# SDFIdk/malstroem

Measured on AMD Instinct MI355X. Metric: Mcells/s fill->D8->accum->label on 16384^2 f32 DEM, higher is better.
Workload: dtype f32 fill / f64 no-flats+D8+accum / u8 flowdir / i32 labels; 1 GPU; 16384x16384 float32 DEM (spectral fBm beta=2 seed 42 (SURVEY 8d recipe)): fill+depths -> no-flats fill -> D8 -> accumulation -> CCL+label_stats -> watersheds+label_count -> pour points; parallelism=1 GPU, one device context, fill_rounds=8, noflat_rounds=84, fill_tiles=70225, fill_visits=44315, fill_cycles=0, noflat_visits=410496, noflat_cycles=410496, nlabels=4637017, fill_algorithm=1, fill_launches=8, noflat_algorithm=2, pour_algorithm=1

## Files before the change

### malstroem_amd/csrc/common.hpp

```cpp
#pragma once
#include <hip/hip_runtime.h>
#include <cstdint>
#include <cstdio>
#include <cstring>
#include <string>
#include <vector>

#include "../../include/malstroem_hip.h"

struct mhip_polygons;
struct mhip_flowpaths;

namespace mh {

void set_error(const char *fmt, ...);
const char *get_error();
const char *dev_env(const char *name);
hipError_t stream_sync(hipStream_t s);
int require_device();

#define MH_HIP(expr)                                                                             \
    do {                                                                                         \
        hipError_t _e = (expr);                                                                  \
        if (_e != hipSuccess) {                                                                  \
            mh::set_error("%s failed: %s (%s:%d)", #expr, hipGetErrorString(_e), __FILE__, __LINE__); \
            return MHIP_EHIP;                                                                    \
        }                                                                                        \
    } while (0)

#define MH_TRY(expr)                \
    do {                            \
        int _rc = (expr);           \
        if (_rc != MHIP_OK) return _rc; \
    } while (0)

#define MH_ARG(cond, msg)                   \
    do {                                    \
        if (!(cond)) {                      \
            mh::set_error("invalid argument: %s", msg); \
            return MHIP_EINVAL;             \
        }                                   \
    } while (0)

int pool_alloc(void **p, size_t bytes);
void pool_free(void *p, size_t bytes);

struct DevBuf {
    void *p = nullptr;
    size_t bytes = 0;
    DevBuf() = default;
    DevBuf(const DevBuf &) = delete;
    DevBuf &operator=(const DevBuf &) = delete;
    ~DevBuf() { release(); }
    int alloc(size_t n)
    {
        if (n == 0) n = 16;
        if (p && bytes >= n && bytes <= 2 * n + 4096) return MHIP_OK;
        release();
        MH_TRY(pool_alloc(&p, n));
        bytes = n;
        return MHIP_OK;
    }
    void release()
    {
        if (p) pool_free(p, bytes);
        p = nullptr;
        bytes = 0;
    }
    template <typename T> T *as() const { return reinterpret_cast<T *>(p); }
};

int upload(DevBuf &b, const void *host, size_t bytes, hipStream_t s);
int download(void *host, const DevBuf &b, size_t bytes, hipStream_t s);
int64_t build_rank_lut(const uint8_t *keep, int64_t nlab, std::vector<int32_t> &lut);
inline bool hyps_res_ok(double res) { return res > 0.0 && res <= 1.7976931348623157e308; }
int trace_on_device(const uint8_t *d_fd, const int32_t *d_lab, int64_t H, int64_t W, const int64_t *cells_rc, int64_t n, int use_bg,
                    int32_t bg, int32_t *out_label, int32_t *out_found, int64_t *out_len, const int64_t *offsets, int64_t *out_cells,
                    hipStream_t s);

__host__ __device__ inline int dir_dr(int k) { return (k == 0 || k == 1 || k == 7) ? -1 : (k >= 3 && k <= 5) ? 1 : 0; }
__host__ __device__ inline int dir_dc(int k) { return (k >= 1 && k <= 3) ? 1 : (k >= 5 && k <= 7) ? -1 : 0; }

__device__ __forceinline__ unsigned d8_code(double z, double u, double ur, double r, double dr, double d, double dl,
                                            double l, double ul)
{
    const double INV_SQRT2 = 0.7071067811865475;
    unsigned i = 8;
    double dzmax = 0.0, dz;
#define MH_D8_STEP(expr, k)          \
    dz = (expr);                     \
    i = dz > dzmax ? (k) : i;        \
    dzmax = fmax(dzmax, dz);
    MH_D8_STEP(__dsub_rn(z, u), 0u)
    MH_D8_STEP(__dmul_rn(__dsub_rn(z, ur), INV_SQRT2), 1u)
    MH_D8_STEP(__dsub_rn(z, r), 2u)
    MH_D8_STEP(__dmul_rn(__dsub_rn(z, dr), INV_SQRT2), 3u)
    MH_D8_STEP(__dsub_rn(z, d), 4u)
    MH_D8_STEP(__dmul_rn(__dsub_rn(z, dl), INV_SQRT2), 5u)
    MH_D8_STEP(__dsub_rn(z, l), 6u)
    MH_D8_STEP(__dmul_rn(__dsub_rn(z, ul), INV_SQRT2), 7u)
#undef MH_D8_STEP
    return i;
}

__device__ __forceinline__ unsigned edge_code(int64_t r, int64_t c, int64_t maxr, int64_t maxc)
{
    unsigned code = 8;
    if (r == 0) code = 0;
    if (r == maxr) code = 4;
    if (c == 0) code = 6;
    if (c == maxc) code = 2;
    if (r == 0 && c == 0) code = 7;
    if (r == 0 && c == maxc) code = 1;
    if (r == maxr && c == 0) code = 5;
    if (r == maxr && c == maxc) code = 3;
    return code;
}

__host__ __device__ inline uint32_t f32_key(float f)
{
    uint32_t u;
    memcpy(&u, &f, 4);
    return (u & 0x80000000u) ? ~u : (u | 0x80000000u);
}
__host__ __device__ inline float key_f32(uint32_t k)
{
    uint32_t u = (k & 0x80000000u) ? (k & 0x7fffffffu) : ~k;
    float f;
    memcpy(&f, &u, 4);
    return f;
}
__device__ __forceinline__ uint32_t dem_key(float v)
{
    if (v != v) return f32_key(__builtin_inff());
    return f32_key(v + 0.0f);
}
__host__ __device__ inline uint64_t f64_key(double f)
{
    uint64_t u;
    memcpy(&u, &f, 8);
    return (u & 0x8000000000000000ull) ? ~u : (u | 0x8000000000000000ull);
}
__host__ __device__ inline double key_f64(uint64_t k)
{
    uint64_t u = (k & 0x8000000000000000ull) ? (k & 0x7fffffffffffffffull) : ~k;
    double f;
    memcpy(&f, &u, 8);
    return f;
}

struct FillStats {
    int32_t rounds = 0;
    int64_t visits = 0;
    int64_t cycles = 0;
    int64_t tiles = 0;
    float hot_ms = 0;
    int32_t hot_launches = 0;
    int32_t algorithm = 0;
    uint32_t overflow = 0;
    bool have_minmax = false, dem_nan = false;
    float dem_min = 0.0f, dem_max = 0.0f;
    int32_t geo_reject = 0;
    int64_t geo_irregular = 0, geo_unreached = 0, geo_mismatch = 0;
};

struct FillRun {
    bool noflat = false;
    const float *dem = nullptr;
    void *out = nullptr;
    int64_t H = 0, W = 0;
    double sh = 0, dg = 0;
    const float *seed = nullptr;
    double seed_add = 0;
    int fixed_top = 0, fixed_bot = 0;
    int rounds_per_batch = 8;
    bool attach_only = false;
    struct Impl;
    Impl *impl;
    FillRun();
    ~FillRun();
    FillRun(const FillRun &) = delete;
    FillRun &operator=(const FillRun &) = delete;
    int begin(hipStream_t s, bool *active);
    int batch(hipStream_t s, bool *active);
    int activate_row(int side, hipStream_t s);
    int attach(hipStream_t s);
    int certify(hipStream_t s, bool *changed);
    int finish(hipStream_t s, FillStats *st);
};
void noflat_seed(FillRun &f, const float *d_filled, double sh, double dg, int64_t ncells_global);
struct PfRun;
struct FillHandover {
    PfRun *run = nullptr;
    const float *dem = nullptr;
    float *filled = nullptr, *depths = nullptr;
    int64_t H = 0, W = 0;
    const uint16_t *bslot = nullptr;
    const uint32_t *tabV = nullptr;
    int ntr = 0, ntc = 0;
    bool pending = false, queued = false, violated = false, repaired = false;
    bool suspect = false;
    unsigned long long *wet = nullptr;
    bool wet_ok = false;
    bool wet_pass = false;
    FillStats st_repair;
    FillHandover() = default;
    FillHandover(const FillHandover &) = delete;
    FillHandover &operator=(const FillHandover &) = delete;
    ~FillHandover();
    void release();
};
int fill_handover_complete(FillHandover *ho, hipStream_t s);
int fill_handover_repair(FillHandover *ho, hipStream_t s);
int fill_plain_dev(const float *d_dem, float *d_out, int64_t H, int64_t W, hipStream_t s, FillStats *st, float *d_depths = nullptr,
                   bool *depths_done = nullptr, FillHandover *ho = nullptr);
int fill_check_f32_dev(const float *d_dem, const float *d_filled, int64_t H, int64_t W, int fixed_top, int fixed_bot, hipStream_t s,
                       unsigned int *d_flag);
int fill_plain_pflood_dev(const float *d_dem, float *d_out, float *d_depths, int64_t H, int64_t W, hipStream_t s, FillStats *st, bool *violated = nullptr,
                          uint32_t *overflow = nullptr, FillHandover *ho = nullptr);
struct PfRun {
    const float *dem = nullptr;
    float *out = nullptr;
    int64_t H = 0, W = 0;
    int fixed_top = 0, fixed_bot = 0;
    uint32_t overflow = 0;
    struct Impl;
    Impl *impl;
    PfRun();
    ~PfRun();
    PfRun(const PfRun &) = delete;
    PfRun &operator=(const PfRun &) = delete;
    int begin(hipStream_t s);
    int halo_changed(int side, hipStream_t s);
    int batch(hipStream_t s);
    int finish(hipStream_t s, float *d_depths, FillStats *st, bool *violated = nullptr, FillHandover *ho = nullptr);
    int finish_late(hipStream_t s, float *d_depths, bool *violated);
    int proof_flag(hipStream_t s, unsigned int *h_flag);
    int solve(hipStream_t s);
    int pack(hipStream_t s, int row0, int nrows);
    int publish_edges(hipStream_t s);
};
struct StageHook {
    enum Point { FIRST_VISIT = 0, TAIL_ROUNDS = 1, FINISH = 3 };
    void (*fn)(void *, hipStream_t) = nullptr;
    void *arg = nullptr;
    bool fired = false;
    int at = TAIL_ROUNDS;
    void fire(hipStream_t s)
    {
        if (fn && !fired) {
            fired = true;
            fn(arg, s);
        }
    }
    void fire_at(int point, hipStream_t s)
    {
        if (point == at) fire(s);
    }
};

struct GeoRun {
    const float *dem = nullptr, *filled = nullptr;
    double *out = nullptr;
    uint32_t *dist = nullptr;
    int64_t H = 0, W = 0;
    double sh = 0, dg = 0;
    int fixed_top = 0, fixed_bot = 0;
    bool allow_partial = false;
    double seed_add = 0;
    bool partial = false;
    StageHook *tail_hook = nullptr;
    uint8_t *d8_out = nullptr;
    unsigned int *d8_nodir = nullptr;
    bool d8_done = false;
    bool defer_out = false;
    bool out_deferred = false;
    FillHandover *handover = nullptr;
    bool wet_used = false;
    struct Impl;
    Impl *impl;
    GeoRun();
    ~GeoRun();
    GeoRun(const GeoRun &) = delete;
    GeoRun &operator=(const GeoRun &) = delete;
    int begin(hipStream_t s, bool *applicable, bool *active);
    int batch(hipStream_t s, bool *active);
    int halo_changed(int side, hipStream_t s);
    int end(hipStream_t s, bool *ok, FillStats *st);
    int launch_rounds(hipStream_t s, int nb);
};
struct D8Sink {
    uint8_t *flowdir = nullptr;
    unsigned int *nodir = nullptr;
    bool done = false;
    uint32_t *dist = nullptr;
    bool defer = false, deferred = false;
};
int noflat_assemble_dev(const float *d_filled, const uint32_t *d_dist, double *d_out, int64_t n, double seed_add, hipStream_t s);
int fill_noflat_geodesic_dev(const float *d_dem, const float *d_filled, double *d_out, int64_t H, int64_t W, double sh, double dg, double seed_add,
                             hipStream_t s, FillStats *st, bool *partial, StageHook *tail_hook = nullptr, D8Sink *d8 = nullptr, FillHandover *ho = nullptr);
int noflat_verify_dev(const float *d_dem, const double *d_out, int64_t H, int64_t W, double sh, double dg, hipStream_t s, bool *ok, int fixed_top = 0,
                      int fixed_bot = 0);
int fill_noflat_dev(const float *d_dem, double *d_out, int64_t H, int64_t W, double sh, double dg, hipStream_t s,
                    FillStats *st = nullptr, const float *d_filled = nullptr, StageHook *tail_hook = nullptr, D8Sink *d8 = nullptr,
                    FillHandover *ho = nullptr);
int short_diag_dev(const float *d_dem, int64_t n, double *sh, double *dg, hipStream_t s);
int depths_dev(const float *d_filled, const float *d_dem, float *d_out, int64_t n, hipStream_t s);
int d8_dev(const double *d_z, uint8_t *d_out, int64_t H, int64_t W, int edges_outward, hipStream_t s, int64_t row_off = 0,
           int64_t Hg = 0, unsigned int *d_interior_nodir = nullptr);
void short_diag_from_minmax(float mn, float mx, bool has_nan, double *sh, double *dg);
int minmax_dev(const float *d_x, int64_t n, float *mn, float *mx, int *has_nan, hipStream_t s);
int row_update_dev(void *d_dst, const void *d_src, int64_t nbytes, int *changed, hipStream_t s);
int copy_bandwidth_dev(size_t bytes, int reps, double *gbs, hipStream_t s);
int read_bandwidth_dev(size_t bytes, int reps, double *gbs, hipStream_t s);
int row_update_async(void *d_dst, const void *d_src, int64_t nbytes, int *d_changed, hipStream_t s);
int trace_downstream_dev(const uint8_t *d_fd, const int32_t *d_lab, int64_t H, int64_t W, const int64_t *d_cells, int64_t n, int use_bg,
// ... 278 lines not shown
```

### malstroem_amd/csrc/ctx.hip

```cpp
#include <mutex>
#include <new>
#include <string>
#include <vector>

#include "ctx.hpp"

namespace mh {

static void drop_hyps(mhip_ctx *c)
{
    c->hyps_total = -1;
    c->have[MHIP_R_FINALDEPTHS] = false;
    c->wetat_events = -1;
    c->wetat_out.release();
}

static void drop_flow_distance(mhip_ctx *c)
{
    std::lock_guard<std::mutex> lk(c->fdist_mu);
    c->fdist_unresolved = -1;
    c->fdist_out.release();
    c->fdist_rec.release();
}

// ... 300 lines not shown
int mhip_ctx_upload_dem(mhip_ctx *c, const float *dem) { return mhip_ctx_upload(c, MHIP_R_DEM, dem); }

int mhip_ctx_upload_rows(mhip_ctx *c, int which, int64_t row0, int64_t nrows, const void *host)
{
    MH_ARG(c && host && which >= 0 && which < MHIP_R_COUNT_ && row0 >= 0 && nrows >= 1 && row0 + nrows <= c->H_owned,
           "ctx_upload_rows(ctx, which, row0, nrows, host)");
    MH_HIP(hipSetDevice(c->device));
    MH_TRY(ctx_raster(c, which));
    MH_TRY(ctx_settle(c, which, true));
    ctx_wrote(c, which, true);
    c->have[which] = false;
    MH_TRY(ctx_copy_rows(c, c->r[which].p, raster_elem(which), row0, nrows, const_cast<void *>(host), hipMemcpyHostToDevice));
    if (row0 + nrows == c->H_owned) {
        c->have[which] = true;
        if (which == MHIP_R_LABELS) c->labels_filtered = true;
    }
    return MHIP_OK;
}

int mhip_ctx_download_rows(mhip_ctx *c, int which, int64_t row0, int64_t nrows, void *host)
{
    MH_ARG(c && host && which >= 0 && which < MHIP_R_COUNT_ && row0 >= 0 && nrows >= 1 && row0 + nrows <= c->H_owned,
           "ctx_download_rows(ctx, which, row0, nrows, host)");
    MH_ARG(c->have[which], "raster has not been computed or uploaded");
    MH_TRY(ctx_settle(c, which, false));
    return ctx_copy_rows(c, c->r[which].p, raster_elem(which), row0, nrows, host, hipMemcpyDeviceToHost);
}

int mhip_ctx_download(mhip_ctx *c, int which, void *host)
{
    MH_ARG(c && host && which >= 0 && which < MHIP_R_COUNT_, "ctx_download(ctx, which, host)");
    return mhip_ctx_download_rows(c, which, 0, c->H_owned, host);
}

int mhip_ctx_trace_downstream(mhip_ctx *c, const int64_t *cells_rc, int64_t n, int use_background, int32_t background, int32_t *out_label,
                              int32_t *out_found, int64_t *out_len, const int64_t *offsets, int64_t *out_cells)
{
    MH_ARG(c && n >= 0 && (n == 0 || cells_rc), "ctx_trace_downstream(ctx, cells, n, ...)");
    MH_ARG(c->have[MHIP_R_FLOWDIR] && c->have[MHIP_R_LABELS], "ctx_trace_downstream needs flow directions and labels");
    MH_ARG(!c->ht && !c->hb, "stream tracing runs on an undivided raster");
    if (n == 0) return MHIP_OK;
    MH_HIP(hipSetDevice(c->device));
    return trace_on_device(c->r[MHIP_R_FLOWDIR].as<uint8_t>(), c->r[MHIP_R_LABELS].as<int32_t>(), c->H, c->W, cells_rc, n, use_background,
                           background, out_label, out_found, out_len, offsets, out_cells, c->stream);
}

int mhip_ctx_sync(mhip_ctx *c)
{
    MH_ARG(c, "ctx");
    MH_HIP(stream_sync(c->stream));
    return MHIP_OK;
}

int mhip_ctx_stage_ms(mhip_ctx *c, int stage, float *ms)
{
    MH_ARG(c && ms, "ctx_stage_ms(ctx, stage, ms)");
    const int k = timer_slot(stage);
    MH_ARG(k >= 0 && c->timers[k].valid, "stage has not been run");
    MH_HIP(hipEventSynchronize(c->timers[k].b));
    MH_HIP(hipEventElapsedTime(ms, c->timers[k].a, c->timers[k].b));
    return MHIP_OK;
}

int mhip_ctx_kernel_ms(mhip_ctx *c, const char *kernel, float *ms_total, int32_t *launches)
{
    MH_ARG(c && kernel && ms_total && launches, "ctx_kernel_ms(ctx, kernel, ms, launches)");
    const std::string k(kernel);
    if (k == "d8") {
        *launches = 1;
        return mhip_ctx_stage_ms(c, MHIP_STAGE_FLOWDIR, ms_total);
    }
    if (k == "d8_steady") {
        MH_ARG(c->have[MHIP_R_NOFLAT] && !c->ht && !c->hb, "d8_steady needs the no-flats surface on an undivided context");
        MH_HIP(hipSetDevice(c->device));
        double *g = nullptr;
        MH_TRY(ctx_noflat(c, &g));
        MH_TRY(ctx_raster(c, MHIP_R_FLOWDIR));
        MH_TRY(c->nodir_cnt.alloc(4));
        constexpr int REPS = 16;
        StageTimer *t;
        MH_TRY(ctx_timer(c, D8_STEADY_SLOT, &t));
        hipStream_t s = c->stream;
        ctx_wrote(c, MHIP_R_FLOWDIR);
        MH_HIP(hipMemsetAsync(c->nodir_cnt.p, 0, 4, s));
        for (int i = 0; i < REPS + 2; ++i) {
            if (i == 2) MH_HIP(hipEventRecord(t->a, s));
            MH_TRY(d8_dev(g, c->r[MHIP_R_FLOWDIR].as<uint8_t>(), c->H, c->W, 1, s, 0, c->H_global, c->nodir_cnt.as<unsigned int>()));
        }
        MH_HIP(hipEventRecord(t->b, s));
        MH_HIP(hipEventSynchronize(t->b));
        MH_HIP(hipEventElapsedTime(ms_total, t->a, t->b));
        c->have[MHIP_R_FLOWDIR] = true;
        c->nodir_valid = true;
        c->flowdir_own = true;
        *launches = REPS;
        return MHIP_OK;
    }
    if (k == "hyps_table" || k == "final_depths") {
        *launches = 1;
        return mhip_ctx_stage_ms(c, k == "hyps_table" ? HYPS_KERNEL_SLOT : FINAL_KERNEL_SLOT, ms_total);
    }
    if (k == "wet_at") {
        *launches = 1;
        return mhip_ctx_stage_ms(c, WETAT_KERNEL_SLOT, ms_total);
    }
    if (k == "fill_round") {
        *launches = c->fill_rounds;
        return mhip_ctx_stage_ms(c, MHIP_STAGE_FILL, ms_total);
    }
    if (k == "noflat_round") {
        *launches = c->noflat_rounds;
        return mhip_ctx_stage_ms(c, MHIP_STAGE_NOFLAT, ms_total);
    }
    set_error("unknown kernel family '%s'", kernel);
    return MHIP_EINVAL;
}

int mhip_ctx_get_i64(mhip_ctx *c, const char *key, int64_t *value)
{
    MH_ARG(c && key && value, "ctx_get_i64(ctx, key, value)");
    const std::string k(key);
    if (k == "nlabels_raw") *value = c->nlabels_raw;
    else if (k == "nlabels") {
        if (c->nlabels < 0 && c->have[MHIP_R_LABELS]) {
            MH_HIP(hipSetDevice(c->device));
            MH_TRY(ctx_label_max(c, c->stream));
        }
        *value = c->nlabels;
    }
    else if (k == "fill_rounds") *value = c->fill_rounds;
    else if (k == "noflat_rounds") *value = c->noflat_rounds;
    else if (k == "fill_visits") *value = c->fill_st.visits;
    else if (k == "fill_cycles") *value = c->fill_st.cycles;
    else if (k == "fill_tiles") *value = c->fill_st.tiles;
    else if (k == "fill_algorithm") *value = c->fill_st.algorithm;
    else if (k == "fill_handover") *value = c->fill_handover;
    else if (k == "wetbits_used") *value = (c->wet_pass_used ? 1 : 0) | (c->wet_label_used ? 2 : 0);
    else if (k == "fill_handover_rechecks") *value = c->fill_handover_rechecks;
    else if (k == "fill_overflow") *value = c->fill_st.overflow;
    else if (k == "fill_launches") *value = c->fill_st.rounds;
    else if (k == "fill_hot_launches") *value = c->fill_st.hot_launches;
    else if (k == "noflat_hot_launches") *value = c->noflat_st.hot_launches;
    else if (k == "accum_algorithm") *value = c->accum_algorithm;
    else if (k == "flowdir_computed") *value = (c->have[MHIP_R_FLOWDIR] && c->flowdir_own) ? 1 : 0;
    else if (k == "pour_algorithm") *value = c->pour_algorithm;
    else if (k == "noflat_algorithm") *value = c->noflat_st.algorithm;
    else if (k == "noflat_pending") *value = c->noflat_pending ? 1 : 0;
    else if (k == "noflat_visits") *value = c->noflat_st.visits;
    else if (k == "noflat_reject") *value = c->noflat_st.geo_reject;
    else if (k == "noflat_reject_irregular") *value = c->noflat_st.geo_irregular;
    else if (k == "noflat_reject_unreached") *value = c->noflat_st.geo_unreached;
    else if (k == "noflat_reject_mismatch") *value = c->noflat_st.geo_mismatch;
    else if (k == "noflat_cycles") *value = c->noflat_st.cycles;
    else if (k == "hyps_bins") *value = c->hyps_total;
    else if (k == "hyps_lds_spills") *value = c->hyps_spills;
    else if (k == "wet_at_events") *value = c->wetat_events;
    else if (k == "flow_distance_unresolved") *value = c->fdist_unresolved;
    else if (k == "hand_undrained") *value = c->hand_undrained;
    else if (k == "reach_catchments") *value = c->rcatch_nreach;
    else if (k == "inundation") *value = c->inund_held;
    else if (k == "zones") *value = c->nzone;
    else if (k == "H") *value = c->H;
    else if (k == "W") *value = c->W;
    else {
        set_error("unknown key '%s'", key);
        return MHIP_EINVAL;
    }
    return MHIP_OK;
}

int mhip_ctx_get_f64(mhip_ctx *c, const char *key, double *value)
{
    MH_ARG(c && key && value, "ctx_get_f64(ctx, key, value)");
    const std::string k(key);
    if (k == "short") *value = c->sh;
    else if (k == "diag") *value = c->dg;
    else if (k == "fill_hot_ms") *value = c->fill_st.hot_ms;
    else if (k == "noflat_hot_ms") *value = c->noflat_st.hot_ms;
    else {
        set_error("unknown key '%s'", key);
        return MHIP_EINVAL;
    }
    return MHIP_OK;
}

int mhip_ctx_raw_stats(mhip_ctx *c, mhip_stat_record *records)
{
    MH_ARG(c && records && c->raw_stats.p && c->nlabels_raw >= 0, "ctx_raw_stats needs a LABEL run");
    return ctx_fetch(c, c->raw_stats, sizeof(mhip_stat_record) * (size_t)(c->nlabels_raw + 1), records);
}

int mhip_ctx_apply_keep(mhip_ctx *c, const uint8_t *keep)
{
    MH_ARG(c, "ctx");
    MH_HIP(hipSetDevice(c->device));
    return ctx_apply_keep_on(c, keep, c->stream);
}

int mhip_ctx_stats(mhip_ctx *c, mhip_stat_record *records)
{
    MH_ARG(c && records && c->stats_valid && c->labels_filtered, "ctx_stats needs LABEL + apply_keep (or mhip_ctx_hyps) on the resident depths and labels");
    return ctx_fetch(c, c->stats, sizeof(mhip_stat_record) * (size_t)(c->nlabels + 1), records);
}

int mhip_ctx_watershed_counts(mhip_ctx *c, int64_t *counts)
{
    MH_ARG(c && counts && c->ws_counts_valid, "ctx_watershed_counts needs a WATERSHED run on the resident labels");
    return ctx_fetch(c, c->ws_counts, 8 * (size_t)(c->nlabels + 1), counts);
}

int mhip_ctx_pourpoints(mhip_ctx *c, mhip_index_record *records)
{
    MH_ARG(c && records && c->pour_valid, "ctx_pourpoints needs a POURPOINTS run on the resident labels and accumulated flow");
    return ctx_fetch(c, c->pour, sizeof(mhip_index_record) * (size_t)(c->nlabels + 1), records);
}

int mhip_ctx_hyps(mhip_ctx *c, double res, int64_t *total)
{
    MH_ARG(c && total && hyps_res_ok(res), "ctx_hyps(ctx, 0 < res < inf, total)");
    MH_ARG(!(c->nranks > 1 || c->ht || c->hb), "hypsometry on a row band is not built (the tables of the bands add up: a later step); use an undivided context");
    MH_ARG(c->have[MHIP_R_DEPTHS] && c->have[MHIP_R_LABELS] && !c->ccl_pending, "ctx_hyps needs the DEPTHS and LABELS rasters");
    MH_ARG(c->labels_filtered, "ctx_hyps needs mhip_ctx_apply_keep after the LABEL run");
    MH_HIP(hipSetDevice(c->device));
    hipStream_t s = c->stream;
    const int64_t n = c->H * c->W;
    c->hyps_total = -1;
    if (!c->stats_valid) {
        MH_TRY(ctx_label_max(c, s));
        MH_TRY(c->stats.alloc(sizeof(mhip_stat_record) * (size_t)(c->nlabels + 1)));
        MH_TRY(label_stats_dev(c->r[MHIP_R_DEPTHS].as<float>(), c->r[MHIP_R_LABELS].as<int32_t>(), n, c->nlabels, c->stats.as<mhip_stat_record>(), s,
                               c->W, c->labels_components));
        c->stats_valid = true;
    }
    const int64_t nlab = c->nlabels;
    MH_TRY(c->hyps_off.alloc(8 * (size_t)(nlab + 2)));
    StageTimer *k;
    MH_TRY(ctx_timer(c, HYPS_KERNEL_SLOT, &k));
    MH_TRY(stage_begin(c, MHIP_STAGE_HYPS, s));
    int64_t tot = 0;
    MH_TRY(hyps_layout_dev(c->stats.as<double>() + 1, 4, nlab, res, c->hyps_off.as<int64_t>(), &tot, s));
    MH_TRY(c->hyps_cnt.alloc(4 * (size_t)tot));
    MH_TRY(c->hyps_sum.alloc(8 * (size_t)tot));
    MH_TRY(hyps_table_dev(c->r[MHIP_R_DEPTHS].as<float>(), c->r[MHIP_R_LABELS].as<int32_t>(), n, c->W, nlab, res, c->hyps_off.as<int64_t>(), tot,
                          c->hyps_cnt.as<uint32_t>(), c->hyps_sum.as<double>(), &c->hyps_spills, s, k->a, k->b));
    MH_TRY(stage_end(c, MHIP_STAGE_HYPS, s));
    k->valid = true;
    c->hyps_total = tot;
    *total = tot;
    return MHIP_OK;
}

int mhip_ctx_hyps_fetch(mhip_ctx *c, int64_t *offsets, int64_t *counts, double *sums)
{
    MH_ARG(c && offsets && counts && sums, "ctx_hyps_fetch(ctx, offsets, counts, sums)");
    MH_ARG(c->hyps_total >= 0, "ctx_hyps_fetch needs mhip_ctx_hyps on the resident depths and labels");
    MH_HIP(hipSetDevice(c->device));
    hipStream_t s = c->stream;
    const size_t tot = (size_t)c->hyps_total;
    std::vector<uint32_t> c32(tot + 1);
    MH_HIP(hipMemcpyAsync(offsets, c->hyps_off.p, 8 * (size_t)(c->nlabels + 2), hipMemcpyDeviceToHost, s));
    if (tot) {
        MH_HIP(hipMemcpyAsync(c32.data(), c->hyps_cnt.p, 4 * tot, hipMemcpyDeviceToHost, s));
        MH_HIP(hipMemcpyAsync(sums, c->hyps_sum.p, 8 * tot, hipMemcpyDeviceToHost, s));
    }
    MH_HIP(stream_sync(s));
    for (size_t k = 0; k < tot; ++k) counts[k] = (int64_t)c32[k];
    return MHIP_OK;
}

int mhip_ctx_final_depths(mhip_ctx *c, const double *q, mhip_final_record *records)
{
    MH_ARG(c && q && records, "ctx_final_depths(ctx, q, records)");
    MH_ARG(c->hyps_total >= 0 && c->stats_valid, "ctx_final_depths needs mhip_ctx_hyps on the resident depths and labels");
    MH_HIP(hipSetDevice(c->device));
    hipStream_t s = c->stream;
    const int64_t nlab = c->nlabels, n = c->H * c->W;
    DevBuf d_q;
    MH_TRY(upload(d_q, q, 8 * (size_t)(nlab + 1), s));
    MH_TRY(c->hyps_rec.alloc(sizeof(mhip_final_record) * (size_t)(nlab + 1)));
    MH_TRY(ctx_raster(c, MHIP_R_FINALDEPTHS));
    c->have[MHIP_R_FINALDEPTHS] = false;
    StageTimer *k;
    MH_TRY(ctx_timer(c, FINAL_KERNEL_SLOT, &k));
    MH_TRY(stage_begin(c, MHIP_STAGE_FINALDEPTHS, s));
    MH_TRY(hyps_levels_dev(nlab, c->hyps_off.as<int64_t>(), c->hyps_cnt.as<uint32_t>(), c->hyps_sum.as<double>(), c->stats.as<double>() + 1, 4,
                           d_q.as<double>(), c->hyps_rec.as<mhip_final_record>(), s));
    MH_TRY(final_depths_dev(c->r[MHIP_R_DEPTHS].as<float>(), c->r[MHIP_R_LABELS].as<int32_t>(), n, c->W, nlab, c->hyps_rec.as<mhip_final_record>(),
                            c->r[MHIP_R_FINALDEPTHS].as<float>(), s, k->a, k->b));
    MH_TRY(stage_end(c, MHIP_STAGE_FINALDEPTHS, s));
    k->valid = true;
    c->have[MHIP_R_FINALDEPTHS] = true;
    return ctx_fetch(c, c->hyps_rec, sizeof(mhip_final_record) * (size_t)(nlab + 1), records);
}

int mhip_ctx_wet_at(mhip_ctx *c, int32_t K, const double *q, const float *values, mhip_final_record *records)
{
    MH_ARG(c && q && values && records, "ctx_wet_at(ctx, K, q, values, records)");
    MH_ARG(wet_at_events_ok(K, values), "ctx_wet_at: 1 to 16 events whose values are finite, > 0 and strictly increasing");
    MH_ARG(!(c->nranks > 1 || c->ht || c->hb), "wet_at on a row band is not built (it needs the bands' hypsometry tables: a later step); use an undivided context");
    MH_ARG(c->hyps_total >= 0 && c->stats_valid, "ctx_wet_at needs mhip_ctx_hyps on the resident depths and labels");
    MH_HIP(hipSetDevice(c->device));
    hipStream_t s = c->stream;
    const int64_t nlab = c->nlabels, n = c->H * c->W;
    const size_t nt = (size_t)K * (size_t)(nlab + 1);
    DevBuf d_q, d_rec;
    MH_TRY(upload(d_q, q, 8 * nt, s));
// ... 277 lines not shown
```

### malstroem_amd/csrc/noflat_geo.hip

```cpp
#include <algorithm>
#include <cmath>
#include <cstdlib>
#include <mutex>
#include <string>
#include <type_traits>
#include <vector>

#include "common.hpp"
#include "handover_addr.hpp"

namespace mh {

namespace {

constexpr int WN = 64;
constexpr int TI = 62;
constexpr uint32_t DINF = 0xE0000000u;
constexpr uint32_t WMAX = 1u << 28;
constexpr uint32_t D_IRR = 0xFFFFFFFFu;
constexpr uint32_t M_NOFLAT = 0xFF00u;
constexpr uint32_t M_IRR = 0xFD00u;
constexpr uint32_t M_WALL = 0xFE00u;
constexpr int DPP_WF_SL1 = 0x130;
constexpr int DPP_WF_SR1 = 0x138;
#ifndef NG_MAXCYC
#define NG_MAXCYC 1
#endif
enum { C_IRREGULAR = 0, C_UNREACHED = 1, C_MISMATCH = 2, C_FATAL = 3, C_PROOF = 4, C_STATS = 8 };
static_assert(WN == ho::WN && TI == ho::TI, "handover_addr.hpp cuts the raster like this file");

__device__ __forceinline__ uint32_t from_left(uint32_t v) { return (uint32_t)__builtin_amdgcn_update_dpp(0, (int)v, DPP_WF_SR1, 0xf, 0xf, true); }
__device__ __forceinline__ uint32_t from_right(uint32_t v) { return (uint32_t)__builtin_amdgcn_update_dpp(0, (int)v, DPP_WF_SL1, 0xf, 0xf, true); }

__device__ __forceinline__ float fleft(float v)
{
    return __int_as_float(__builtin_amdgcn_update_dpp(0x7f800000, __float_as_int(v), DPP_WF_SR1, 0xf, 0xf, false));
}
__device__ __forceinline__ float fright(float v)
{
    return __int_as_float(__builtin_amdgcn_update_dpp(0x7f800000, __float_as_int(v), DPP_WF_SL1, 0xf, 0xf, false));
}

__device__ __forceinline__ uint32_t class_above(float V)
{
    const uint32_t b = __float_as_uint(V), ex = (b >> 23) & 0xffu;
    const uint32_t e = ((b >> 31) && (b & 0x7fffffu) == 0u) ? ex - 1u : ex;
    return (ex == 0u || ex == 255u) ? 255u : e;
}
__device__ __forceinline__ double class_ulp(uint32_t e) { return __longlong_as_double((long long)(e + 1023u - 127u - 52u) << 52); }

struct GeoArgs {
    int64_t H, W;
    int ntr, ntc, nt;
    const float *F;
    uint32_t *d;
    uint32_t *blk;
    uint32_t *hdr;
    uint8_t *mark;
    const int *list;
    const uint32_t *count;
    const uint32_t *tab;
    unsigned long long *counters;
    int maxcyc;
    int append, round_next;
    int *amark;
    int *list_next;
    uint32_t *count_next;
    int fixed_top, fixed_bot;
    const float *ho_dem;
    const uint16_t *ho_bslot;
    const uint32_t *ho_tabV;
    float *ho_F, *ho_depths;
    unsigned long long *ho_wet;
};

template <int R> __device__ __forceinline__ void lds_put(uint32_t addr, uint32_t v) { asm volatile("ds_write_b32 %0, %1 offset:%2" : : "v"(addr), "v"(v), "n"(R) : "memory"); }
template <int R> __device__ __forceinline__ uint32_t lds_get(uint32_t addr)
{
    uint32_t v;
    asm volatile("ds_read_b32 %0, %1 offset:%2" : "=v"(v) : "v"(addr), "n"(R) : "memory");
    return v;
}
__device__ __forceinline__ void lds_wait() { asm volatile("s_waitcnt lgkmcnt(0)" : : : "memory"); }
template <int R0, int N> __device__ __forceinline__ void lds_put_rows(uint32_t addr, const uint32_t (&x)[WN])
{
    if constexpr (N > 0) {
        lds_put<R0 * (WN + 1) * 4>(addr, x[R0]);
        lds_put_rows<R0 + 1, N - 1>(addr, x);
    }
}
template <int R0, int N> __device__ __forceinline__ void lds_get_rows(uint32_t addr, uint32_t (&x)[WN])
{
    if constexpr (N > 0) {
        x[R0] = lds_get<R0 * (WN + 1) * 4>(addr);
        lds_get_rows<R0 + 1, N - 1>(addr, x);
    }
}
template <int C0, int N> __device__ __forceinline__ void lds_get_cols(uint32_t addr, uint32_t (&x)[WN])
{
    if constexpr (N > 0) {
        x[C0] = lds_get<C0 * 4>(addr);
        lds_get_cols<C0 + 1, N - 1>(addr, x);
    }
}
__device__ __forceinline__ void transpose32(uint32_t (&x)[WN], uint32_t scr_b, int lane)
{
    lds_put_rows<0, WN>(scr_b + 4u * lane, x);
    lds_wait();
    lds_get_cols<0, WN>(scr_b + 4u * (WN + 1) * lane, x);
    lds_wait();
#pragma unroll
    for (int c = 0; c < WN; ++c) asm volatile("" : "+v"(x[c]));
}

struct LaneW {
    __device__ __forceinline__ void get(uint32_t mword, const uint32_t *tab_l, uint32_t &s, uint32_t &g) const
    {
        const uint32_t e = (mword >> 8) & 0xffu;
        s = tab_l[e];
        g = tab_l[256 + e];
    }
};

template <bool DOWN, typename WT>
__device__ __forceinline__ void pass(uint32_t (&d)[WN], uint32_t (&ni)[WN], const WT wt, const uint32_t *tab_l, uint32_t &acc_all,
                                     uint32_t &acc_first, uint32_t &acc_last)
{
    constexpr int first = DOWN ? 1 : TI, dir = DOWN ? 1 : -1;
    constexpr int bC = DOWN ? 0 : 4, bL = DOWN ? 7 : 5, bR = DOWN ? 1 : 3;
#pragma unroll
    for (int r = 0; r < WN; ++r) asm volatile("" : "+v"(d[r]), "+v"(ni[r]));
#pragma unroll
    for (int i = 0; i < TI; ++i) {
        const int r = first + dir * i;
        const uint32_t behind = d[r - dir];
        const uint32_t bl = from_left(behind), br = from_right(behind);
        const uint32_t w = ni[r];
        uint32_t S, G;
        wt.get(w, tab_l, S, G);
        const uint32_t c0 = (behind + S) | (uint32_t)__builtin_amdgcn_sbfe((int)w, bC, 1);
        const uint32_t c1 = (bl + G) | (uint32_t)__builtin_amdgcn_sbfe((int)w, bL, 1);
        const uint32_t c2 = (br + G) | (uint32_t)__builtin_amdgcn_sbfe((int)w, bR, 1);
        const uint32_t cu = d[r];
        const uint32_t nv = min(min(c0, c1), min(c2, cu));
        const uint32_t x = nv ^ cu;
        acc_all |= x;
        asm volatile("" : "+v"(acc_all));
        if (r == 1) acc_first |= (w & 0x83u) != 0x83u ? x : 0u;
        if (r == TI) acc_last |= (w & 0x38u) != 0x38u ? x : 0u;
        d[r] = nv;
        __builtin_amdgcn_sched_barrier(0);
    }
}

template <typename WT>
__device__ __forceinline__ void relax(uint32_t (&d)[WN], uint32_t (&ni)[WN], const WT wt, const uint32_t *tab_l, uint32_t scr_b, int lane, int maxcyc,
                                      unsigned &wake, bool &changed, bool &capped, unsigned &cycles)
{
    const uint64_t INNER = ((1ull << TI) - 1) << 1, B1 = 2ull, B62 = 1ull << TI;
    capped = true;
#pragma nounroll
    for (int cyc = 0; cyc < maxcyc; ++cyc) {
        uint64_t chg = 0;
        ++cycles;
#pragma nounroll
        for (int half = 0; half < 2; ++half) {
            uint32_t acc_all = 0, acc_first = 0, acc_last = 0;
            pass<true>(d, ni, wt, tab_l, acc_all, acc_first, acc_last);
            pass<false>(d, ni, wt, tab_l, acc_all, acc_first, acc_last);
            const uint64_t all = __ballot(acc_all != 0), fst = __ballot(acc_first != 0), lst = __ballot(acc_last != 0);
            chg |= all;
            const unsigned e_first = (fst & INNER) ? 1u : 0u, e_last = (lst & INNER) ? 1u : 0u;
            const unsigned l1 = (all & B1) ? 1u : 0u, l62 = (all & B62) ? 1u : 0u;
            const unsigned f1 = (fst & B1) ? 1u : 0u, f62 = (fst & B62) ? 1u : 0u, g1 = (lst & B1) ? 1u : 0u, g62 = (lst & B62) ? 1u : 0u;
            if (half == 0)
                wake |= (e_first << 1) | (e_last << 7) | (l1 << 3) | (l62 << 5) | (f1 << 0) | (f62 << 2) | (g1 << 6) | (g62 << 8);
            else
                wake |= (e_first << 3) | (e_last << 5) | (l1 << 1) | (l62 << 7) | (f1 << 0) | (f62 << 6) | (g1 << 2) | (g62 << 8);
            transpose32(d, scr_b, lane);
#pragma unroll
            for (int r = 0; r < WN; ++r) ni[r] = __builtin_amdgcn_alignbit(ni[r], ni[r], 16);
        }
        changed |= chg != 0;
        if (!chg) {
            capped = false;
            break;
        }
    }
}

constexpr int NMK = 9;
#define NG_DPP " row_mask:0xf bank_mask:0xf bound_ctrl:1\n\t"
#define NG_ROW(O, I, B, BIT)                                                                                                                 \
    "v_add_u32 %[u], %[" B "], %[S]\n\t"                                                                                                    \
    "v_add_u32_dpp %[t], %[" B "], %[G] wave_shr:1" NG_DPP                                                                                   \
    "v_add_u32_dpp %[k], %[" B "], %[G] wave_shl:1" NG_DPP                                                                                   \
    "v_min3_u32 %[t], %[u], %[t], %[k]\n\t"                                                                                                 \
    "v_bfe_i32 %[k], %[m], " BIT ", 1\n\t"                                                                                                  \
    "v_min_u32 %[" O "], %[t], %[" I "]\n\t"                                                                                                \
    "v_bfi_b32 %[" O "], %[k], %[" I "], %[" O "]\n\t"                                                                                      \
    "v_bitop3_b32 %[acc], %[" O "], %[acc], %[" I "] bitop3:0xde\n\t"
template <int R, int DIR>
__device__ __forceinline__ void rows6_wl(uint32_t (&d)[WN], const uint32_t m, const uint32_t S, const uint32_t G, uint32_t &acc)
{
    static_assert((R >> 5) == ((R + 5 * DIR) >> 5), "one mask word a block");
    uint32_t o0, o1, o2, o3, o4, o5, u, t, k;
    if constexpr (DIR > 0)
        asm volatile(NG_ROW("o0", "i0", "b", "%[bit]") NG_ROW("o1", "i1", "o0", "%[bit]+1") NG_ROW("o2", "i2", "o1", "%[bit]+2")
                     NG_ROW("o3", "i3", "o2", "%[bit]+3") NG_ROW("o4", "i4", "o3", "%[bit]+4") NG_ROW("o5", "i5", "o4", "%[bit]+5")
                     : [o0] "=&v"(o0), [o1] "=&v"(o1), [o2] "=&v"(o2), [o3] "=&v"(o3), [o4] "=&v"(o4), [o5] "=&v"(o5), [u] "=&v"(u), [t] "=&v"(t),
                       [k] "=&v"(k), [acc] "+v"(acc)
                     : [b] "v"(d[R - DIR]), [i0] "v"(d[R]), [i1] "v"(d[R + DIR]), [i2] "v"(d[R + 2 * DIR]), [i3] "v"(d[R + 3 * DIR]),
                       [i4] "v"(d[R + 4 * DIR]), [i5] "v"(d[R + 5 * DIR]), [S] "v"(S), [G] "v"(G), [m] "v"(m), [bit] "n"(R & 31));
    else
        asm volatile(NG_ROW("o0", "i0", "b", "%[bit]") NG_ROW("o1", "i1", "o0", "%[bit]-1") NG_ROW("o2", "i2", "o1", "%[bit]-2")
                     NG_ROW("o3", "i3", "o2", "%[bit]-3") NG_ROW("o4", "i4", "o3", "%[bit]-4") NG_ROW("o5", "i5", "o4", "%[bit]-5")
                     : [o0] "=&v"(o0), [o1] "=&v"(o1), [o2] "=&v"(o2), [o3] "=&v"(o3), [o4] "=&v"(o4), [o5] "=&v"(o5), [u] "=&v"(u), [t] "=&v"(t),
                       [k] "=&v"(k), [acc] "+v"(acc)
                     : [b] "v"(d[R - DIR]), [i0] "v"(d[R]), [i1] "v"(d[R + DIR]), [i2] "v"(d[R + 2 * DIR]), [i3] "v"(d[R + 3 * DIR]),
                       [i4] "v"(d[R + 4 * DIR]), [i5] "v"(d[R + 5 * DIR]), [S] "v"(S), [G] "v"(G), [m] "v"(m), [bit] "n"(R & 31));
    d[R] = o0; d[R + DIR] = o1; d[R + 2 * DIR] = o2; d[R + 3 * DIR] = o3; d[R + 4 * DIR] = o4; d[R + 5 * DIR] = o5;
}
template <int R, int DIR>
__device__ __forceinline__ uint32_t row1_wl(uint32_t (&d)[WN], const uint32_t m, const uint32_t S, const uint32_t G, uint32_t &acc)
{
    uint32_t o0, u, t, k;
    const uint32_t cu = d[R];
    asm volatile("s_nop 1\n\t" NG_ROW("o0", "i0", "b", "%[bit]") "s_nop 1"
                 : [o0] "=&v"(o0), [u] "=&v"(u), [t] "=&v"(t), [k] "=&v"(k), [acc] "+v"(acc)
                 : [b] "v"(d[R - DIR]), [i0] "v"(cu), [S] "v"(S), [G] "v"(G), [m] "v"(m), [bit] "n"(R & 31));
    d[R] = o0;
    return o0 ^ cu;
}
template <int R, int DIR, int N>
__device__ __forceinline__ void blocks_wl(uint32_t (&d)[WN], const uint32_t lo, const uint32_t hi, const uint32_t S, const uint32_t G, uint32_t &acc)
{
    if constexpr (N > 0) {
        rows6_wl<R, DIR>(d, R < 32 ? lo : hi, S, G, acc);
        __builtin_amdgcn_sched_barrier(0);
        blocks_wl<R + 6 * DIR, DIR, N - 1>(d, lo, hi, S, G, acc);
    }
}
template <bool DOWN>
__device__ __forceinline__ void pass_wl(uint32_t (&d)[WN], const uint32_t imm_lo, const uint32_t imm_hi, const uint32_t S, const uint32_t G,
                                        const bool edge_first, const bool edge_last, uint32_t &acc_all, uint32_t &acc_first, uint32_t &acc_last)
{
#pragma unroll
    for (int r = 0; r < WN; ++r) asm volatile("" : "+v"(d[r]));
    uint32_t lo = imm_lo, hi = imm_hi;
    asm volatile("" : "+v"(lo), "+v"(hi));
    if constexpr (DOWN) {
        const uint32_t x1 = row1_wl<1, 1>(d, lo, S, G, acc_all);
        acc_first |= edge_first ? x1 : 0u;
        __builtin_amdgcn_sched_barrier(0);
        blocks_wl<2, 1, 10>(d, lo, hi, S, G, acc_all);
        const uint32_t x2 = row1_wl<TI, 1>(d, hi, S, G, acc_all);
        acc_last |= edge_last ? x2 : 0u;
    } else {
        const uint32_t x2 = row1_wl<TI, -1>(d, hi, S, G, acc_all);
        acc_last |= edge_last ? x2 : 0u;
        __builtin_amdgcn_sched_barrier(0);
        blocks_wl<TI - 1, -1, 10>(d, lo, hi, S, G, acc_all);
        const uint32_t x1 = row1_wl<1, -1>(d, lo, S, G, acc_all);
        acc_first |= edge_first ? x1 : 0u;
    }
    __builtin_amdgcn_sched_barrier(0);
}

__device__ __forceinline__ void relax_wl(uint32_t (&d)[WN], const uint32_t (&mk)[13], const uint32_t S, const uint32_t G, uint32_t scr_b, int lane, int maxcyc,
                                         unsigned &wake, bool &changed, bool &capped, unsigned &cycles)
{
    const uint64_t INNER = ((1ull << TI) - 1) << 1, B1 = 2ull, B62 = 1ull << TI;
    capped = true;
#pragma nounroll
    for (int cyc = 0; cyc < maxcyc; ++cyc) {
        uint64_t chg = 0;
        ++cycles;
        {
            uint32_t acc_all = 0, acc_first = 0, acc_last = 0;
            pass_wl<true>(d, mk[0], mk[1], S, G, (mk[8] & 1u) != 0u, (mk[8] & 2u) != 0u, acc_all, acc_first, acc_last);
            pass_wl<false>(d, mk[0], mk[1], S, G, (mk[8] & 1u) != 0u, (mk[8] & 2u) != 0u, acc_all, acc_first, acc_last);
            const uint64_t all = __ballot(acc_all != 0), fst = __ballot(acc_first != 0), lst = __ballot(acc_last != 0);
            chg |= all;
            const unsigned e_first = (fst & INNER) ? 1u : 0u, e_last = (lst & INNER) ? 1u : 0u;
            const unsigned l1 = (all & B1) ? 1u : 0u, l62 = (all & B62) ? 1u : 0u;
            const unsigned f1 = (fst & B1) ? 1u : 0u, f62 = (fst & B62) ? 1u : 0u, g1 = (lst & B1) ? 1u : 0u, g62 = (lst & B62) ? 1u : 0u;
            wake |= (e_first << 1) | (e_last << 7) | (l1 << 3) | (l62 << 5) | (f1 << 0) | (f62 << 2) | (g1 << 6) | (g62 << 8);
            transpose32(d, scr_b, lane);
        }
        {
            uint32_t acc_all = 0, acc_first = 0, acc_last = 0;
            pass_wl<true>(d, mk[4], mk[5], S, G, (mk[8] & 4u) != 0u, (mk[8] & 8u) != 0u, acc_all, acc_first, acc_last);
            pass_wl<false>(d, mk[4], mk[5], S, G, (mk[8] & 4u) != 0u, (mk[8] & 8u) != 0u, acc_all, acc_first, acc_last);
            const uint64_t all = __ballot(acc_all != 0), fst = __ballot(acc_first != 0), lst = __ballot(acc_last != 0);
            chg |= all;
            const unsigned e_first = (fst & INNER) ? 1u : 0u, e_last = (lst & INNER) ? 1u : 0u;
            const unsigned l1 = (all & B1) ? 1u : 0u, l62 = (all & B62) ? 1u : 0u;
            const unsigned f1 = (fst & B1) ? 1u : 0u, f62 = (fst & B62) ? 1u : 0u, g1 = (lst & B1) ? 1u : 0u, g62 = (lst & B62) ? 1u : 0u;
            wake |= (e_first << 3) | (e_last << 5) | (l1 << 1) | (l62 << 7) | (f1 << 0) | (f62 << 6) | (g1 << 2) | (g62 << 8);
            transpose32(d, scr_b, lane);
        }
        changed |= chg != 0;
        if (!chg) {
            capped = false;
            break;
        }
    }
}

constexpr int NMK2 = 13;
#define NG_ROW2(O, I, B, BIT)                                                                                                                \
    "v_bfe_i32 %[k], %[c], " BIT ", 1\n\t"                                                                                                  \
    "v_bfi_b32 %[g], %[k], %[G2], %[G1]\n\t"                                                                                                \
    "v_bfi_b32 %[s], %[k], %[S2], %[S1]\n\t"                                                                                                \
    "v_add_u32 %[u], %[" B "], %[s]\n\t"                                                                                                    \
    "v_add_u32_dpp %[t], %[" B "], %[g] wave_shr:1" NG_DPP                                                                                   \
    "v_add_u32_dpp %[k], %[" B "], %[g] wave_shl:1" NG_DPP                                                                                   \
    "v_min3_u32 %[t], %[u], %[t], %[k]\n\t"                                                                                                 \
    "v_bfe_i32 %[k], %[m], " BIT ", 1\n\t"                                                                                                  \
    "v_min_u32 %[" O "], %[t], %[" I "]\n\t"                                                                                                \
    "v_bfi_b32 %[" O "], %[k], %[" I "], %[" O "]\n\t"                                                                                      \
    "v_bitop3_b32 %[acc], %[" O "], %[acc], %[" I "] bitop3:0xde\n\t"
struct TwoWeights {
    uint32_t S1, G1, S2, G2;
};
template <int R, int DIR>
__device__ __forceinline__ void rows6_wl2(uint32_t (&d)[WN], const uint32_t m, const uint32_t c, const TwoWeights w, uint32_t &acc)
{
    static_assert((R >> 5) == ((R + 5 * DIR) >> 5), "one mask word a block");
    uint32_t o0, o1, o2, o3, o4, o5, u, t, k, sw, gw;
    if constexpr (DIR > 0)
        asm volatile(NG_ROW2("o0", "i0", "b", "%[bit]") NG_ROW2("o1", "i1", "o0", "%[bit]+1") NG_ROW2("o2", "i2", "o1", "%[bit]+2")
                     NG_ROW2("o3", "i3", "o2", "%[bit]+3") NG_ROW2("o4", "i4", "o3", "%[bit]+4") NG_ROW2("o5", "i5", "o4", "%[bit]+5")
                     : [o0] "=&v"(o0), [o1] "=&v"(o1), [o2] "=&v"(o2), [o3] "=&v"(o3), [o4] "=&v"(o4), [o5] "=&v"(o5), [u] "=&v"(u), [t] "=&v"(t),
                       [k] "=&v"(k), [s] "=&v"(sw), [g] "=&v"(gw), [acc] "+v"(acc)
                     : [b] "v"(d[R - DIR]), [i0] "v"(d[R]), [i1] "v"(d[R + DIR]), [i2] "v"(d[R + 2 * DIR]), [i3] "v"(d[R + 3 * DIR]),
                       [i4] "v"(d[R + 4 * DIR]), [i5] "v"(d[R + 5 * DIR]), [S1] "v"(w.S1), [G1] "v"(w.G1), [S2] "v"(w.S2), [G2] "v"(w.G2), [m] "v"(m),
                       [c] "v"(c), [bit] "n"(R & 31));
    else
        asm volatile(NG_ROW2("o0", "i0", "b", "%[bit]") NG_ROW2("o1", "i1", "o0", "%[bit]-1") NG_ROW2("o2", "i2", "o1", "%[bit]-2")
                     NG_ROW2("o3", "i3", "o2", "%[bit]-3") NG_ROW2("o4", "i4", "o3", "%[bit]-4") NG_ROW2("o5", "i5", "o4", "%[bit]-5")
                     : [o0] "=&v"(o0), [o1] "=&v"(o1), [o2] "=&v"(o2), [o3] "=&v"(o3), [o4] "=&v"(o4), [o5] "=&v"(o5), [u] "=&v"(u), [t] "=&v"(t),
                       [k] "=&v"(k), [s] "=&v"(sw), [g] "=&v"(gw), [acc] "+v"(acc)
                     : [b] "v"(d[R - DIR]), [i0] "v"(d[R]), [i1] "v"(d[R + DIR]), [i2] "v"(d[R + 2 * DIR]), [i3] "v"(d[R + 3 * DIR]),
                       [i4] "v"(d[R + 4 * DIR]), [i5] "v"(d[R + 5 * DIR]), [S1] "v"(w.S1), [G1] "v"(w.G1), [S2] "v"(w.S2), [G2] "v"(w.G2), [m] "v"(m),
                       [c] "v"(c), [bit] "n"(R & 31));
    d[R] = o0; d[R + DIR] = o1; d[R + 2 * DIR] = o2; d[R + 3 * DIR] = o3; d[R + 4 * DIR] = o4; d[R + 5 * DIR] = o5;
}
template <int R, int DIR>
__device__ __forceinline__ uint32_t row1_wl2(uint32_t (&d)[WN], const uint32_t m, const uint32_t c, const TwoWeights w, uint32_t &acc)
{
    uint32_t o0, u, t, k, sw, gw;
    const uint32_t cu = d[R];
    asm volatile("s_nop 1\n\t" NG_ROW2("o0", "i0", "b", "%[bit]") "s_nop 1"
                 : [o0] "=&v"(o0), [u] "=&v"(u), [t] "=&v"(t), [k] "=&v"(k), [s] "=&v"(sw), [g] "=&v"(gw), [acc] "+v"(acc)
                 : [b] "v"(d[R - DIR]), [i0] "v"(cu), [S1] "v"(w.S1), [G1] "v"(w.G1), [S2] "v"(w.S2), [G2] "v"(w.G2), [m] "v"(m), [c] "v"(c),
                   [bit] "n"(R & 31));
    d[R] = o0;
    return o0 ^ cu;
}
template <int R, int DIR, int N>
__device__ __forceinline__ void blocks_wl2(uint32_t (&d)[WN], const uint32_t lo, const uint32_t hi, const uint32_t clo, const uint32_t chi, const TwoWeights w,
                                           uint32_t &acc)
{
    if constexpr (N > 0) {
        rows6_wl2<R, DIR>(d, R < 32 ? lo : hi, R < 32 ? clo : chi, w, acc);
        __builtin_amdgcn_sched_barrier(0);
        blocks_wl2<R + 6 * DIR, DIR, N - 1>(d, lo, hi, clo, chi, w, acc);
    }
}
template <bool DOWN>
__device__ __forceinline__ void pass_wl2(uint32_t (&d)[WN], const uint32_t imm_lo, const uint32_t imm_hi, const uint32_t cls_lo, const uint32_t cls_hi,
                                         const TwoWeights w, const bool edge_first, const bool edge_last, uint32_t &acc_all, uint32_t &acc_first,
                                         uint32_t &acc_last)
{
#pragma unroll
    for (int r = 0; r < WN; ++r) asm volatile("" : "+v"(d[r]));
    uint32_t lo = imm_lo, hi = imm_hi, clo = cls_lo, chi = cls_hi;
    asm volatile("" : "+v"(lo), "+v"(hi), "+v"(clo), "+v"(chi));
    if constexpr (DOWN) {
        const uint32_t x1 = row1_wl2<1, 1>(d, lo, clo, w, acc_all);
        acc_first |= edge_first ? x1 : 0u;
        __builtin_amdgcn_sched_barrier(0);
        blocks_wl2<2, 1, 10>(d, lo, hi, clo, chi, w, acc_all);
        const uint32_t x2 = row1_wl2<TI, 1>(d, hi, chi, w, acc_all);
        acc_last |= edge_last ? x2 : 0u;
    } else {
        const uint32_t x2 = row1_wl2<TI, -1>(d, hi, chi, w, acc_all);
        acc_last |= edge_last ? x2 : 0u;
        __builtin_amdgcn_sched_barrier(0);
        blocks_wl2<TI - 1, -1, 10>(d, lo, hi, clo, chi, w, acc_all);
        const uint32_t x1 = row1_wl2<1, -1>(d, lo, clo, w, acc_all);
        acc_first |= edge_first ? x1 : 0u;
    }
    __builtin_amdgcn_sched_barrier(0);
}
__device__ __forceinline__ void relax_wl2(uint32_t (&d)[WN], const uint32_t (&mk)[NMK2], const TwoWeights w, uint32_t scr_b, int lane, int maxcyc, unsigned &wake,
                                          bool &changed, bool &capped, unsigned &cycles)
{
    const uint64_t INNER = ((1ull << TI) - 1) << 1, B1 = 2ull, B62 = 1ull << TI;
    capped = true;
#pragma nounroll
    for (int cyc = 0; cyc < maxcyc; ++cyc) {
        uint64_t chg = 0;
        ++cycles;
        {
            uint32_t acc_all = 0, acc_first = 0, acc_last = 0;
            pass_wl2<true>(d, mk[0], mk[1], mk[9], mk[10], w, (mk[8] & 1u) != 0u, (mk[8] & 2u) != 0u, acc_all, acc_first, acc_last);
            pass_wl2<false>(d, mk[0], mk[1], mk[9], mk[10], w, (mk[8] & 1u) != 0u, (mk[8] & 2u) != 0u, acc_all, acc_first, acc_last);
            const uint64_t all = __ballot(acc_all != 0), fst = __ballot(acc_first != 0), lst = __ballot(acc_last != 0);
            chg |= all;
            const unsigned e_first = (fst & INNER) ? 1u : 0u, e_last = (lst & INNER) ? 1u : 0u;
            const unsigned l1 = (all & B1) ? 1u : 0u, l62 = (all & B62) ? 1u : 0u;
            const unsigned f1 = (fst & B1) ? 1u : 0u, f62 = (fst & B62) ? 1u : 0u, g1 = (lst & B1) ? 1u : 0u, g62 = (lst & B62) ? 1u : 0u;
            wake |= (e_first << 1) | (e_last << 7) | (l1 << 3) | (l62 << 5) | (f1 << 0) | (f62 << 2) | (g1 << 6) | (g62 << 8);
            transpose32(d, scr_b, lane);
        }
        {
            uint32_t acc_all = 0, acc_first = 0, acc_last = 0;
            pass_wl2<true>(d, mk[4], mk[5], mk[11], mk[12], w, (mk[8] & 4u) != 0u, (mk[8] & 8u) != 0u, acc_all, acc_first, acc_last);
            pass_wl2<false>(d, mk[4], mk[5], mk[11], mk[12], w, (mk[8] & 4u) != 0u, (mk[8] & 8u) != 0u, acc_all, acc_first, acc_last);
            const uint64_t all = __ballot(acc_all != 0), fst = __ballot(acc_first != 0), lst = __ballot(acc_last != 0);
            chg |= all;
            const unsigned e_first = (fst & INNER) ? 1u : 0u, e_last = (lst & INNER) ? 1u : 0u;
            const unsigned l1 = (all & B1) ? 1u : 0u, l62 = (all & B62) ? 1u : 0u;
            const unsigned f1 = (fst & B1) ? 1u : 0u, f62 = (fst & B62) ? 1u : 0u, g1 = (lst & B1) ? 1u : 0u, g62 = (lst & B62) ? 1u : 0u;
            wake |= (e_first << 3) | (e_last << 5) | (l1 << 1) | (l62 << 7) | (f1 << 0) | (f62 << 6) | (g1 << 2) | (g62 << 8);
            transpose32(d, scr_b, lane);
        }
        changed |= chg != 0;
        if (!chg) {
            capped = false;
            break;
        }
    }
}

#define NG_ROW_OPEN(O, I, B)                                                                                                                 \
    "v_add_u32 %[u], %[" B "], %[S]\n\t"                                                                                                    \
    "v_add_u32_dpp %[t], %[" B "], %[G] wave_shr:1" NG_DPP                                                                                   \
    "v_add_u32_dpp %[k], %[" B "], %[G] wave_shl:1" NG_DPP                                                                                   \
    "v_min3_u32 %[t], %[u], %[t], %[k]\n\t"                                                                                                 \
    "v_min_u32 %[" O "], %[t], %[" I "]\n\t"                                                                                                \
    "v_cndmask_b32_e64 %[" O "], %[" O "], %[" I "], %[ring]\n\t"                                                                            \
    "v_bitop3_b32 %[acc], %[" O "], %[acc], %[" I "] bitop3:0xde\n\t"
template <int R, int DIR>
__device__ __forceinline__ void rows6_open(uint32_t (&d)[WN], const uint64_t ring, const uint32_t S, const uint32_t G, uint32_t &acc)
{
    uint32_t o0, o1, o2, o3, o4, o5, u, t, k;
    asm volatile(NG_ROW_OPEN("o0", "i0", "b") NG_ROW_OPEN("o1", "i1", "o0") NG_ROW_OPEN("o2", "i2", "o1") NG_ROW_OPEN("o3", "i3", "o2")
                 NG_ROW_OPEN("o4", "i4", "o3") NG_ROW_OPEN("o5", "i5", "o4")
                 : [o0] "=&v"(o0), [o1] "=&v"(o1), [o2] "=&v"(o2), [o3] "=&v"(o3), [o4] "=&v"(o4), [o5] "=&v"(o5), [u] "=&v"(u), [t] "=&v"(t), [k] "=&v"(k),
                   [acc] "+v"(acc)
                 : [b] "v"(d[R - DIR]), [i0] "v"(d[R]), [i1] "v"(d[R + DIR]), [i2] "v"(d[R + 2 * DIR]), [i3] "v"(d[R + 3 * DIR]), [i4] "v"(d[R + 4 * DIR]),
                   [i5] "v"(d[R + 5 * DIR]), [S] "v"(S), [G] "v"(G), [ring] "s"(ring));
    d[R] = o0; d[R + DIR] = o1; d[R + 2 * DIR] = o2; d[R + 3 * DIR] = o3; d[R + 4 * DIR] = o4; d[R + 5 * DIR] = o5;
}
template <int R, int DIR>
__device__ __forceinline__ uint32_t row1_open(uint32_t (&d)[WN], const uint64_t ring, const uint32_t S, const uint32_t G, uint32_t &acc)
{
    uint32_t o0, u, t, k;
    const uint32_t cu = d[R];
    asm volatile("s_nop 1\n\t" NG_ROW_OPEN("o0", "i0", "b") "s_nop 1"
                 : [o0] "=&v"(o0), [u] "=&v"(u), [t] "=&v"(t), [k] "=&v"(k), [acc] "+v"(acc)
                 : [b] "v"(d[R - DIR]), [i0] "v"(cu), [S] "v"(S), [G] "v"(G), [ring] "s"(ring));
    d[R] = o0;
    return o0 ^ cu;
}
template <int R, int DIR, int N>
__device__ __forceinline__ void blocks_open(uint32_t (&d)[WN], const uint64_t ring, const uint32_t S, const uint32_t G, uint32_t &acc)
{
    if constexpr (N > 0) {
        rows6_open<R, DIR>(d, ring, S, G, acc);
        __builtin_amdgcn_sched_barrier(0);
        blocks_open<R + 6 * DIR, DIR, N - 1>(d, ring, S, G, acc);
    }
}
template <bool DOWN>
__device__ __forceinline__ void pass_open(uint32_t (&d)[WN], const uint32_t S, const uint32_t G, const bool ring_lane, uint32_t &acc_all, uint32_t &acc_first,
                                          uint32_t &acc_last)
{
#pragma unroll
    for (int r = 0; r < WN; ++r) asm volatile("" : "+v"(d[r]));
    const uint64_t ring = __ballot(ring_lane);
    if constexpr (DOWN) {
        acc_first |= row1_open<1, 1>(d, ring, S, G, acc_all);
        __builtin_amdgcn_sched_barrier(0);
        blocks_open<2, 1, 10>(d, ring, S, G, acc_all);
        acc_last |= row1_open<TI, 1>(d, ring, S, G, acc_all);
    } else {
        acc_last |= row1_open<TI, -1>(d, ring, S, G, acc_all);
        __builtin_amdgcn_sched_barrier(0);
        blocks_open<TI - 1, -1, 10>(d, ring, S, G, acc_all);
        acc_first |= row1_open<1, -1>(d, ring, S, G, acc_all);
    }
    __builtin_amdgcn_sched_barrier(0);
}

__device__ __forceinline__ void relax_open(uint32_t (&d)[WN], const uint32_t S, const uint32_t G, uint32_t scr_b, int lane, int maxcyc, unsigned &wake,
                                           bool &changed, bool &capped, unsigned &cycles)
{
    const uint64_t INNER = ((1ull << TI) - 1) << 1, B1 = 2ull, B62 = 1ull << TI;
    const bool ring_lane = (lane == 0) | (lane == WN - 1);
    capped = true;
#pragma nounroll
    for (int cyc = 0; cyc < maxcyc; ++cyc) {
        uint64_t chg = 0;
        ++cycles;
#pragma nounroll
        for (int half = 0; half < 2; ++half) {
            uint32_t acc_all = 0, acc_first = 0, acc_last = 0;
            pass_open<true>(d, S, G, ring_lane, acc_all, acc_first, acc_last);
            pass_open<false>(d, S, G, ring_lane, acc_all, acc_first, acc_last);
            const uint64_t all = __ballot(acc_all != 0), fst = __ballot(acc_first != 0), lst = __ballot(acc_last != 0);
            chg |= all;
            const unsigned e_first = (fst & INNER) ? 1u : 0u, e_last = (lst & INNER) ? 1u : 0u;
            const unsigned l1 = (all & B1) ? 1u : 0u, l62 = (all & B62) ? 1u : 0u;
            const unsigned f1 = (fst & B1) ? 1u : 0u, f62 = (fst & B62) ? 1u : 0u, g1 = (lst & B1) ? 1u : 0u, g62 = (lst & B62) ? 1u : 0u;
            if (half == 0) wake |= (e_first << 1) | (e_last << 7) | (l1 << 3) | (l62 << 5) | (f1 << 0) | (f62 << 2) | (g1 << 6) | (g62 << 8);
            else wake |= (e_first << 3) | (e_last << 5) | (l1 << 1) | (l62 << 7) | (f1 << 0) | (f62 << 6) | (g1 << 2) | (g62 << 8);
            transpose32(d, scr_b, lane);
        }
        changed |= chg != 0;
        if (!chg) {
            capped = false;
            break;
        }
    }
}

constexpr uint32_t HDR_ACTIVE = 1u << 31, HDR_UNIFORM = 1u << 9, HDR_OPEN = 1u << 10, HDR_TWO = 1u << 11;
template <bool FIRST, bool HANDOVER = false>
__device__ __forceinline__ void visit(const GeoArgs &a, int t, const uint32_t *tab_l, uint32_t scr_b, int lane, unsigned &visits, unsigned &cycles)
{
#ifdef NG_PROFILE
    const long long tp0 = __builtin_amdgcn_s_memtime();
#endif
    const int64_t H = a.H, W = a.W;
    const int ti = t / a.ntc, tj = t - ti * a.ntc;
    const int64_t r0 = (int64_t)ti * TI, c0 = (int64_t)tj * TI;
    const int64_t cc = c0 + lane;
    const bool col_in = cc < W;
    const uint32_t lane_c = (uint32_t)(col_in ? lane : W - 1 - c0);

    const int64_t org = r0 * W + c0;
    const __amdgpu_buffer_rsrc_t rd = __builtin_amdgcn_make_buffer_rsrc((void *)(a.d + org), 0, 0x7fffffff, 0x00020000);
    const __amdgpu_buffer_rsrc_t rb = __builtin_amdgcn_make_buffer_rsrc((void *)(a.blk + (int64_t)t * (WN * WN)), 0, WN * WN * 4, 0x00020000);
    int Wi = (int)W;
    asm volatile("" : "+s"(Wi));
    const int last_row = (int)(H - 1 - r0 < WN - 1 ? H - 1 - r0 : WN - 1);
    uint32_t ni[WN], d[WN], mk[NMK2];
    uint32_t hdr;
    if constexpr (FIRST) {
        const __amdgpu_buffer_rsrc_t rf = __builtin_amdgcn_make_buffer_rsrc((void *)(a.F + org), 0, 0x7fffffff, 0x00020000);
        const bool ring_lane = (lane == 0) | (lane == WN - 1);
        const bool lane_in = (lane >= 1) & (lane <= TI) & (cc < W - 1);
        const bool lane_border = (tj == 0 && lane == 0) | (cc >= W - 1);
        const float PINF = __builtin_inff();
        const int border_row = (int)(H - 1 - r0 < 2 * WN ? H - 1 - r0 : 2 * WN);
        uint32_t lake_any = 0, nirr = 0, nfatal = 0;
        uint32_t proof_bad = 0;
        auto classify = [&](auto inner_tag) {
            constexpr bool INNER = decltype(inner_tag)::value;
            const bool lane_in_c = INNER ? ((lane >= 1) & (lane <= TI)) : lane_in;
            float f[WN];
            uint32_t raised[2] = {0u, 0u};
            if constexpr (!HANDOVER) {
                int so = 0;
#pragma unroll
                for (int r = 0; r < WN; ++r) {
                    f[r] = __uint_as_float(__builtin_amdgcn_raw_buffer_load_b32(rf, (int)((INNER ? (uint32_t)lane : lane_c) * 4u), INNER ? r * Wi * 4 : so * 4, 0));
                    so = r < last_row ? so + Wi : so;
                }
            } else {
                const ho::Win w = ho::window(H, W, a.ntr, a.ntc, ti, tj);
                const int64_t tab0 = ho::tab_origin(w), tab_left = ho::tab_words_behind_origin(w) * 4;
                const __amdgpu_buffer_rsrc_t re = __builtin_amdgcn_make_buffer_rsrc((void *)(a.ho_dem + org), 0, 0x7fffffff, 0x00020000);
                const __amdgpu_buffer_rsrc_t rs = __builtin_amdgcn_make_buffer_rsrc((void *)(a.ho_bslot + org), 0, 0x7fffffff, 0x00020000);
                const __amdgpu_buffer_rsrc_t rt =
                    __builtin_amdgcn_make_buffer_rsrc((void *)(a.ho_tabV + tab0), 0, (int)(tab_left < 0x7fffffff ? tab_left : 0x7fffffff), 0x00020000);
                const __amdgpu_buffer_rsrc_t rF = __builtin_amdgcn_make_buffer_rsrc((void *)(a.ho_F + org), 0, 0x7fffffff, 0x00020000);
                const __amdgpu_buffer_rsrc_t rD =
                    __builtin_amdgcn_make_buffer_rsrc((void *)(a.ho_depths ? a.ho_depths + org : a.ho_F), 0, a.ho_depths ? 0x7fffffff : 0, 0x00020000);
                const uint32_t col_read = INNER ? (uint32_t)lane : (uint32_t)ho::col_of(w, lane);
                const bool bcol = INNER ? false : ho::border_col(w, lane);
                const uint32_t lane_bytes = ho::tab_lane_words(w, lane) * 4u;
                const int row_bytes_top = (int)(ho::tab_row_words(w, 0) * 4u), row_bytes_mid = (int)(ho::tab_row_words(w, 1) * 4u),
                          row_bytes_bot = (int)(ho::tab_row_words(w, WN - 1) * 4u);
                const bool ocol = INNER ? lane_in_c : ho::own_col(w, lane);
                volatile __attribute__((address_space(3))) uint32_t *const scr_p = (volatile __attribute__((address_space(3))) uint32_t *)(uintptr_t)scr_b + lane;
                uint32_t below = 0u;
                constexpr int QR = 16;
                uint32_t sl[WN];
                auto load_q = [&](int q) {
#pragma unroll
                    for (int r = q * QR; r < (q + 1) * QR; ++r) {
                        const int so = INNER ? r * Wi : (r < last_row ? r : last_row) * Wi;
                        f[r] = __uint_as_float(__builtin_amdgcn_raw_buffer_load_b32(re, (int)(col_read * 4u), so * 4, 0));
                        sl[r] = (uint32_t)(uint16_t)__builtin_amdgcn_raw_buffer_load_b16(rs, (int)(col_read * 2u), so * 2, 0);
                    }
                    __builtin_amdgcn_sched_barrier(0);
                };
                auto gather_q = [&](int q) {
#pragma unroll
                    for (int r = q * QR; r < (q + 1) * QR; ++r) {
                        const bool border = INNER ? false : (bcol | ho::border_row(w, r));
                        sl[r] = __builtin_amdgcn_raw_buffer_load_b32(rt, (int)(lane_bytes + ho::tab_slot(sl[r], border) * 4u),
                                                                     r == 0 ? row_bytes_top : (r == WN - 1 ? row_bytes_bot : row_bytes_mid), 0);
                    }
                    __builtin_amdgcn_sched_barrier(0);
                };
                auto finish_q = [&](int q) {
#pragma unroll
                    for (int r = q * QR; r < (q + 1) * QR; ++r) {
                        const bool border = INNER ? false : (bcol | ho::border_row(w, r));
                        const float e = f[r];
                        const float lev = key_f32(max(dem_key(e), sl[r]));
                        const float v = border ? e : lev;
                        raised[r >> 5] |= v > e ? 1u << (r & 31) : 0u;
                        below |= v < e ? 1u : 0u;
                        asm volatile("" : "+v"(below), "+v"(raised[r >> 5]));
                        if ((INNER ? (r >= 1 && r <= TI) : ho::own_row(w, r)) && ocol) {
                            __builtin_amdgcn_raw_buffer_store_b32(__float_as_uint(v), rF, lane * 4, r * Wi * 4, 0);
                            __builtin_amdgcn_raw_buffer_store_b32(__float_as_uint(v - e), rD, lane * 4, r * Wi * 4, 0);
                        }
                        scr_p[r * (WN + 1)] = __float_as_uint(v);
                        __builtin_amdgcn_sched_barrier(0);
                    }
                };
                load_q(0);
                load_q(1);
                gather_q(0);
                load_q(2);
                gather_q(1);
                finish_q(0);
                load_q(3);
                gather_q(2);
                finish_q(1);
                gather_q(3);
                finish_q(2);
                finish_q(3);
                proof_bad |= below;
                asm volatile("" : "+v"(raised[0]), "+v"(raised[1]));
                {
                    const int64_t wet_left = ho::wet_bytes_behind(w);
                    const __amdgpu_buffer_rsrc_t rW = __builtin_amdgcn_make_buffer_rsrc(
                        (void *)(a.ho_wet ? a.ho_wet + ho::wet_index(w, 0) : (unsigned long long *)a.ho_F), 0,
                        a.ho_wet ? (int)(wet_left < 0x7fffffff ? wet_left : 0x7fffffff) : 0, 0x00020000);
                    typedef uint32_t u32x2 __attribute__((ext_vector_type(2)));
                    const u32x2 word = {raised[0], raised[1]};
                    if (ocol) __builtin_amdgcn_raw_buffer_store_b64(word, rW, lane * 8, 0, 0);
                }
                lds_wait();
                __builtin_amdgcn_sched_barrier(0);
                lds_get_rows<0, WN>(scr_b + 4u * lane, sl);
                lds_wait();
#pragma unroll
                for (int r = 0; r < WN; ++r) {
                    asm volatile("" : "+v"(sl[r]));
                    f[r] = __uint_as_float(sl[r]);
                }
                __builtin_amdgcn_sched_barrier(0);
            }
            float upl = PINF, up = PINF, upr = PINF, cul = fleft(f[0]), cur = fright(f[0]);
            float h_up = PINF, h_cu = fminf(fminf(cul, f[0]), cur);
            uint32_t e_cu = class_above(f[0]), tv_cu = tab_l[e_cu & 0xffu];
#pragma unroll
            for (int r = 0; r < WN; ++r) {
                const float V = f[r], dn = r + 1 < WN ? f[r + 1] : PINF;
                const float dnl = r + 1 < WN ? fleft(dn) : PINF, dnr = r + 1 < WN ? fright(dn) : PINF;
                const float h_dn = fminf(fminf(dnl, dn), dnr);
                const bool lower = fminf(fminf(h_up, h_dn), fminf(cul, cur)) < V;
                h_up = h_cu;
                h_cu = h_dn;
                const bool border = INNER ? false : (lane_border | (ti == 0 && r == 0 && !a.fixed_top) | (r == border_row && !a.fixed_bot) | (r > border_row));
                const bool src = lower | border;
                const bool ring = (r == 0) | (r == WN - 1) | ring_lane | (INNER ? false : (r >= border_row));
                const uint32_t adj = (up == V ? 1u : 0u) | (upr == V ? 2u : 0u) | (cur == V ? 4u : 0u) | (dnr == V ? 8u : 0u) |
                                     (dn == V ? 16u : 0u) | (dnl == V ? 32u : 0u) | (cul == V ? 64u : 0u) | (upl == V ? 128u : 0u);
                const uint32_t e = e_cu, tv = tv_cu;
                e_cu = r + 1 < WN ? class_above(dn) : 255u;
                tv_cu = tab_l[e_cu & 0xffu];
                const bool cell = lane_in_c & !border & !ring;
                const bool flat = cell & !src;
                const bool regular = flat & (adj != 0u) & (e < 253u) & (tv != 0u);
                const bool nan = cell & (V != V);
                const bool irregular = flat & !regular & !nan;
// ... 85 lines not shown
            lds_put_rows<0, WN>(scr_b + 4u * lane, tw);
            lds_wait();
            lds_get_cols<0, 32>(scr_b + 4u * (WN + 1) * lane, tw);
            lds_wait();
#pragma unroll
            for (int r = 0; r < 32; ++r) {
                asm volatile("" : "+v"(tw[r]));
                ni[r] = (ni[r] | (tw[r] << 16)) ^ 0x00ff00ffu;
            }
            lds_get_cols<32, 32>(scr_b + 4u * (WN + 1) * lane, tw);
            lds_wait();
#pragma unroll
            for (int r = 32; r < WN; ++r) {
                asm volatile("" : "+v"(tw[r]));
                ni[r] = (ni[r] | (tw[r] << 16)) ^ 0x00ff00ffu;
            }
        }
        __builtin_amdgcn_sched_barrier(0);
        auto fresh = [&]() {
#pragma unroll
            for (int r = 0; r < WN; ++r) asm volatile("" : "+v"(ni[r]));
        };
        uint32_t esel = 255u;
        fresh();
#pragma unroll
        for (int r = 1; r <= TI; ++r) esel = (ni[r] & 0xffu) != 0xffu ? (ni[r] >> 8) & 0xffu : esel;
        const uint64_t has = __ballot(esel != 255u);
        const uint32_t eref = (uint32_t)__builtin_amdgcn_readlane((int)esel, (int)__builtin_ctzll(has));
        uint32_t mism = 0;
        fresh();
#pragma unroll
        for (int r = 1; r <= TI; ++r) mism |= (ni[r] & 0xffu) != 0xffu ? ((ni[r] >> 8) & 0xffu) ^ eref : 0u;
        unsigned seams = 1u << 4;
        bool open_tile = false;
        {
            uint32_t l_or = 0xffu;
            fresh();
#pragma unroll
            for (int r = 1; r <= TI; ++r) l_or &= ni[r];
            uint32_t any_gap = 0;
#pragma unroll
            for (int r = 1; r <= TI; ++r) any_gap |= ni[r] & 0xffu;
            open_tile = (__ballot(any_gap != 0u) & (((1ull << TI) - 1) << 1)) == 0ull;
            const uint64_t top = __ballot((ni[1] & 0x83u) != 0x83u), bot = __ballot((ni[TI] & 0x38u) != 0x38u);
            const uint64_t lft = __ballot((l_or & 0xe0u) != 0xe0u), rgt = __ballot((l_or & 0x0eu) != 0x0eu);
            const uint64_t INNER = ((1ull << TI) - 1) << 1, B1 = 2ull, B62 = 1ull << TI;
            seams |= (top & INNER) ? 1u << 1 : 0u;
            seams |= (bot & INNER) ? 1u << 7 : 0u;
            seams |= (lft & B1) ? 1u << 3 : 0u;
            seams |= (rgt & B62) ? 1u << 5 : 0u;
            const uint64_t tl = __ballot((ni[1] & 0x80u) == 0u), tr = __ballot((ni[1] & 0x02u) == 0u);
            const uint64_t bl = __ballot((ni[TI] & 0x20u) == 0u), br = __ballot((ni[TI] & 0x08u) == 0u);
            seams |= (tl & B1) ? 1u << 0 : 0u;
            seams |= (tr & B62) ? 1u << 2 : 0u;
            seams |= (bl & B1) ? 1u << 6 : 0u;
            seams |= (br & B62) ? 1u << 8 : 0u;
        }
        const bool uniform = !__any(mism != 0u);
        uint32_t two = 0, c2v = 0;
        if (!uniform) {
            uint32_t e2 = 255u;
            fresh();
#pragma unroll
            for (int r = 1; r <= TI; ++r) {
                const uint32_t e = (ni[r] >> 8) & 0xffu;
                e2 = ((ni[r] & 0xffu) != 0xffu && e != eref) ? e : e2;
            }
            const uint64_t has2 = __ballot(e2 != 255u);
            const uint32_t c2 = (uint32_t)__builtin_amdgcn_readlane((int)e2, (int)__builtin_ctzll(has2 ? has2 : 1ull));
            uint32_t m2 = 0;
            fresh();
#pragma unroll
            for (int r = 1; r <= TI; ++r) {
                const uint32_t e = (ni[r] >> 8) & 0xffu;
                m2 |= ((ni[r] & 0xffu) != 0xffu && e != eref && e != c2) ? 1u : 0u;
            }
            const int delta = (int)c2 - (int)eref;
            if (has2 && !__any(m2 != 0u) && delta >= -64 && delta < 64) two = HDR_TWO | ((uint32_t)(delta + 64) << 24);
            c2v = c2;
        }
        hdr = HDR_ACTIVE | seams | (uniform ? HDR_UNIFORM : 0u) | ((uniform && open_tile) ? HDR_OPEN : 0u) | (eref << 16) | two;
        __builtin_amdgcn_sched_barrier(0);
        if ((uniform && !open_tile) || two) {
            uint32_t mk[NMK2] = {0u, 0u, 0u, 0u, 0u, 0u, 0u, 0u, 0u, 0u, 0u, 0u, 0u};
            fresh();
#pragma unroll
            for (int r = 0; r < WN; ++r) {
                const uint32_t w = ni[r], bit = 1u << (r & 31);
                const int h = r >> 5;
                mk[0 + h] |= (w & 0xffu) == 0xffu ? bit : 0u;
                mk[2 + h] |= (w & 0xff00u) == M_WALL ? bit : 0u;
                mk[4 + h] |= (w & 0xff0000u) == 0xff0000u ? bit : 0u;
                mk[6 + h] |= (w >> 24) == (M_WALL >> 8) ? bit : 0u;
                if (two) {
                    mk[9 + h] |= ((w & 0xffu) != 0xffu && ((w >> 8) & 0xffu) == c2v) ? bit : 0u;
                    mk[11 + h] |= ((w & 0xff0000u) != 0xff0000u && (w >> 24) == c2v) ? bit : 0u;
                }
            }
            mk[8] = ((ni[1] & 0x83u) != 0x83u ? 1u : 0u) | ((ni[TI] & 0x38u) != 0x38u ? 2u : 0u) |
                    ((ni[1] & 0x830000u) != 0x830000u ? 4u : 0u) | ((ni[TI] & 0x380000u) != 0x380000u ? 8u : 0u);
#pragma unroll
            for (int k = 0; k < NMK; ++k) __builtin_amdgcn_raw_buffer_store_b32(mk[k], rb, lane * 4, k * WN * 4, 0);
            if (two) {
#pragma unroll
                for (int k = NMK; k < NMK2; ++k) __builtin_amdgcn_raw_buffer_store_b32(mk[k], rb, lane * 4, k * WN * 4, 0);
            }
        } else if (!uniform) {
#pragma unroll
            for (int r = 0; r < WN; ++r) __builtin_amdgcn_raw_buffer_store_b32(ni[r], rb, lane * 4, r * WN * 4, 0);
        }
        if (lane == 0) {
            a.hdr[t] = hdr;
            a.mark[t] = 1;
        }
        return;
    } else {
        const uint32_t hdr_m = a.hdr[t];
        if (last_row == WN - 1) {
#pragma unroll
            for (int r = 0; r < WN; ++r) d[r] = __builtin_amdgcn_raw_buffer_load_b32(rd, (int)(lane_c * 4u), r * Wi * 4, 0);
        } else {
            int so = 0;
#pragma unroll
            for (int r = 0; r < WN; ++r) {
                d[r] = __builtin_amdgcn_raw_buffer_load_b32(rd, (int)(lane_c * 4u), so * 4, 0);
                so = r < last_row ? so + Wi : so;
            }
        }
        __builtin_amdgcn_sched_barrier(0);
        hdr = __builtin_amdgcn_readfirstlane(hdr_m);
        if (!(hdr & HDR_ACTIVE)) return;
        if (hdr & HDR_OPEN) {
        } else if (hdr & HDR_UNIFORM) {
#pragma unroll
            for (int k = 0; k < NMK; ++k) mk[k] = __builtin_amdgcn_raw_buffer_load_b32(rb, lane * 4, k * WN * 4, 0);
        } else if (hdr & HDR_TWO) {
#pragma unroll
            for (int k = 0; k < NMK2; ++k) mk[k] = __builtin_amdgcn_raw_buffer_load_b32(rb, lane * 4, k * WN * 4, 0);
        } else {
#pragma unroll
            for (int r = 0; r < WN; ++r) ni[r] = __builtin_amdgcn_raw_buffer_load_b32(rb, lane * 4, r * WN * 4, 0);
        }
    }
    ++visits;
    __builtin_amdgcn_sched_barrier(0);
#ifdef NG_PROFILE
    const long long tp1 = __builtin_amdgcn_s_memtime();
    asm volatile("s_waitcnt vmcnt(0)" ::: "memory");
    const long long tp2 = __builtin_amdgcn_s_memtime();
#endif
    const uint32_t eref = (hdr >> 16) & 0xffu;
    unsigned wake = 0;
    bool changed = false, capped = false;
    if (hdr & HDR_OPEN) relax_open(d, tab_l[eref], tab_l[256 + eref], scr_b, lane, a.maxcyc, wake, changed, capped, cycles);
    else if (hdr & HDR_UNIFORM) {
#pragma unroll
        for (int r = 0; r < WN; ++r) d[r] |= (uint32_t)__builtin_amdgcn_sbfe((int)mk[2 + (r >> 5)], r & 31, 1) & DINF;
        relax_wl(d, mk, tab_l[eref], tab_l[256 + eref], scr_b, lane, a.maxcyc, wake, changed, capped, cycles);
        if (changed) {
#pragma unroll
            for (int r = 1; r <= TI; ++r) d[r] &= ~(uint32_t)__builtin_amdgcn_sbfe((int)mk[2 + (r >> 5)], r & 31, 1);
        }
    }
    else if (hdr & HDR_TWO) {
        const uint32_t c2 = (eref + ((hdr >> 24) & 0x7fu) - 64u) & 0xffu;
#pragma unroll
        for (int r = 0; r < WN; ++r) d[r] |= (uint32_t)__builtin_amdgcn_sbfe((int)mk[2 + (r >> 5)], r & 31, 1) & DINF;
        relax_wl2(d, mk, TwoWeights{tab_l[eref], tab_l[256 + eref], tab_l[c2], tab_l[256 + c2]}, scr_b, lane, a.maxcyc, wake, changed, capped, cycles);
        if (changed) {
#pragma unroll
            for (int r = 1; r <= TI; ++r) d[r] &= ~(uint32_t)__builtin_amdgcn_sbfe((int)mk[2 + (r >> 5)], r & 31, 1);
        }
    } else relax(d, ni, LaneW{}, tab_l, scr_b, lane, a.maxcyc, wake, changed, capped, cycles);
    wake &= hdr & 0x1ffu;
#ifdef NG_PROFILE
    const long long tp3 = __builtin_amdgcn_s_memtime();
#endif

    if (changed) {
        const bool lane_ok = (lane >= 1) & (lane <= TI) & (cc < W - 1);
        if (lane_ok) {
            if (last_row == WN - 1) {
#pragma unroll
                for (int r = 1; r <= TI; ++r) __builtin_amdgcn_raw_buffer_store_b32(d[r], rd, lane * 4, r * Wi * 4, 0);
            } else {
#pragma unroll
                for (int r = 1; r <= TI; ++r)
                    if (r < last_row) __builtin_amdgcn_raw_buffer_store_b32(d[r], rd, lane * 4, r * Wi * 4, 0);
            }
        }
    }
    if (capped) wake |= 1u << 4;
    if (wake) {
        const int p = ti + lane / 3 - 1, q = tj + lane % 3 - 1;
        const bool mine = lane < 9 && ((wake >> lane) & 1u) && p >= 0 && p < a.ntr && q >= 0 && q < a.ntc;
        const int tp = p * a.ntc + q;
        if (!FIRST && a.append) {
            bool fresh = false;
            if (mine) fresh = atomicMax(&a.amark[tp], a.round_next) < a.round_next;
            const uint64_t bal = __ballot(fresh);
            if (bal) {
                uint32_t base = 0;
                if (lane == 0) base = atomicAdd(a.count_next, (uint32_t)__builtin_popcountll(bal));
                base = (uint32_t)__builtin_amdgcn_readfirstlane((int)base);
                if (fresh) a.list_next[base + (uint32_t)__builtin_popcountll(bal & ((1ull << lane) - 1ull))] = tp;
            }
        } else if (mine) {
            a.mark[tp] = 1;
        }
    }
#ifdef NG_PROFILE
    if (!FIRST) {
        asm volatile("s_waitcnt vmcnt(0)" ::: "memory");
        const long long tp4 = __builtin_amdgcn_s_memtime();
        if (lane == 0) {
            const int o = C_STATS + 128 + ((hdr & HDR_OPEN) ? 8 : 0);
            atomicAdd(&a.counters[o + 0], 1ull);
            atomicAdd(&a.counters[o + 1], (unsigned long long)(tp1 - tp0));
            atomicAdd(&a.counters[o + 2], (unsigned long long)(tp2 - tp1));
            atomicAdd(&a.counters[o + 3], (unsigned long long)(tp3 - tp2));
            atomicAdd(&a.counters[o + 4], (unsigned long long)(tp4 - tp3));
        }
    }
#endif
}

template <bool FIRST, int WPB = 4, bool HANDOVER = false>
__device__ __forceinline__ void round_body(const GeoArgs &a)
{
    extern __shared__ __attribute__((aligned(16))) uint32_t lds[];
    const int lane = threadIdx.x & 63;
    const int wave = __builtin_amdgcn_readfirstlane(threadIdx.x >> 6);
    const uint32_t scr_b = (uint32_t)(uintptr_t)(__attribute__((address_space(3))) uint32_t *)(lds + wave * (WN * (WN + 1)));
    uint32_t *tab_l = lds + WPB * (WN * (WN + 1));
    const int nwaves = (int)gridDim.x * WPB, gw = (int)blockIdx.x * WPB + wave;
    uint32_t tw[512 / (64 * WPB)];
#pragma unroll
    for (int k = 0; k < 512 / (64 * WPB); ++k) tw[k] = a.tab[threadIdx.x + k * 64 * WPB];
    const int n = FIRST ? a.nt : (int)__builtin_amdgcn_readfirstlane((int)*a.count);
    const int t_first = FIRST ? 0 : a.list[gw < a.nt ? gw : a.nt - 1];
#pragma unroll
    for (int k = 0; k < 512 / (64 * WPB); ++k) tab_l[threadIdx.x + k * 64 * WPB] = tw[k];
    __syncthreads();
    unsigned visits = 0, cycles = 0;
    for (int i = gw; i < n; i += nwaves) {
        const int t = FIRST ? i : __builtin_amdgcn_readfirstlane(i == gw ? t_first : a.list[i]);
        visit<FIRST, HANDOVER>(a, t, tab_l, scr_b, lane, visits, cycles);
    }
    if (lane == 0 && visits) {
        unsigned long long *st = a.counters + C_STATS + 2 * (gw & 63);
        atomicAdd(&st[0], (unsigned long long)visits);
        atomicAdd(&st[1], (unsigned long long)cycles);
    }
}
__global__ __launch_bounds__(256, 2) void ng_first_kernel(GeoArgs a) { round_body<true>(a); }
__global__ __launch_bounds__(256, 2) void ng_round_kernel(GeoArgs a) { round_body<false>(a); }
__global__ __launch_bounds__(64, 2) void ng_round_w1_kernel(GeoArgs a) { round_body<false, 1>(a); }
__global__ __launch_bounds__(256, 2) void ng_handover_kernel(GeoArgs a) { round_body<true, 4, true>(a); }

__global__ __launch_bounds__(256) void ng_compact_kernel(unsigned long long *mark8, int nwords, int *list, uint32_t *count)
{
    __shared__ uint32_t n_l, base_l;
    if (threadIdx.x == 0) n_l = 0;
    __syncthreads();
    const int w = (int)blockIdx.x * 256 + (int)threadIdx.x;
    const unsigned long long v = w < nwords ? mark8[w] : 0ull;
    unsigned k = 0;
    uint32_t o = 0;
    if (v) {
        mark8[w] = 0;
#pragma unroll
        for (int j = 0; j < 8; ++j) k += ((v >> (8 * j)) & 0xffull) ? 1u : 0u;
        o = atomicAdd(&n_l, k);
    }
    __syncthreads();
    if (threadIdx.x == 0) base_l = n_l ? atomicAdd(count, n_l) : 0u;
    __syncthreads();
    if (v) {
        o += base_l;
#pragma unroll
        for (int j = 0; j < 8; ++j)
            if ((v >> (8 * j)) & 0xffull) list[o++] = 8 * w + j;
    }
}

__device__ __forceinline__ double ng_value(float f, uint32_t dd, double seed_add, bool *beyond)
{
    *beyond = false;
    if (dd == D_IRR) return (double)f + seed_add;
    if (dd >= 0x80000000u) {
        *beyond = true;
        return (double)f + seed_add;
    }
    return dd ? (double)f + (double)dd * class_ulp(class_above(f)) : (double)f;
}

__global__ __launch_bounds__(256) void ng_assemble_kernel(const float *__restrict__ F, const uint32_t *__restrict__ d, double *__restrict__ G, int64_t n,
                                                          double seed_add, unsigned long long *counters)
{
    const int64_t i0 = ((int64_t)blockIdx.x * 256 + threadIdx.x) * 4;
    if (i0 >= n) return;
    unsigned bad = 0;
    auto value = [&](float f, uint32_t dd) {
        bool beyond;
        const double v = ng_value(f, dd, seed_add, &beyond);
        bad += beyond ? 1u : 0u;
        return v;
    };
    if (i0 + 4 <= n) {
        const float4 f = *reinterpret_cast<const float4 *>(F + i0);
        const uint4 dv = *reinterpret_cast<const uint4 *>(d + i0);
        typedef double __attribute__((ext_vector_type(2))) v2d;
        *reinterpret_cast<v2d *>(G + i0) = v2d{value(f.x, dv.x), value(f.y, dv.y)};
        *reinterpret_cast<v2d *>(G + i0 + 2) = v2d{value(f.z, dv.z), value(f.w, dv.w)};
    } else {
        for (int64_t i = i0; i < n; ++i) G[i] = value(F[i], d[i]);
    }
    if (bad && counters) atomicAdd(&counters[C_UNREACHED], (unsigned long long)bad);
}

constexpr int VRB = 16;
__global__ __launch_bounds__(256) void ng_verify_kernel(const float *__restrict__ dem, const double *__restrict__ G, int64_t H, int64_t W, double sh,
                                                        double dg, int fixed_top, int fixed_bot, unsigned long long *counters)
{
    const int64_t c = (int64_t)blockIdx.x * 256 + threadIdx.x;
    const int64_t rb = (int64_t)blockIdx.y * VRB;
    if (c >= W) return;
    const double PINF = __builtin_inf();
    const bool cl = c > 0, cr = c + 1 < W;
    auto row = [&](int64_t r, double (&v)[3]) {
        const bool in = r >= 0 && r < H;
        const double *p = G + (in ? r : 0) * W + c;
        v[0] = (in && cl) ? p[-1] : PINF;
        v[1] = in ? p[0] : PINF;
        v[2] = (in && cr) ? p[1] : PINF;
    };
    double a[3], b[3], n[3];
    row(rb - 1, a);
    row(rb, b);
    unsigned bad = 0;
#pragma unroll 4
    for (int i = 0; i < VRB; ++i) {
        const int64_t r = rb + i;
        if (r >= H) break;
        row(r + 1, n);
        const double own = b[1], dv = (double)dem[r * W + c];
        double want = dv;
        if (r > 0 && r < H - 1 && cl && cr) {
            const double md = fmin(fmin(a[0], a[2]), fmin(n[0], n[2])) + dg;
            const double me = fmin(fmin(a[1], b[0]), fmin(b[2], n[1])) + sh;
            want = fmax(fmin(md, me), dv);
        }
        const bool halo = (r == 0 && fixed_top) || (r == H - 1 && fixed_bot);
        bad += (own == want || halo) ? 0u : 1u;
#pragma unroll
        for (int k = 0; k < 3; ++k) {
            a[k] = b[k];
            b[k] = n[k];
        }
    }
    if (bad) atomicAdd(&counters[C_MISMATCH], (unsigned long long)bad);
}

constexpr int FRB = 32;
__device__ __forceinline__ double dleft(double v)
{
    const uint64_t b = (uint64_t)__double_as_longlong(v);
    const uint32_t lo = from_left((uint32_t)b), hi = from_left((uint32_t)(b >> 32));
    return __longlong_as_double((long long)(((uint64_t)hi << 32) | lo));
}
__device__ __forceinline__ double dright(double v)
{
    const uint64_t b = (uint64_t)__double_as_longlong(v);
    const uint32_t lo = from_right((uint32_t)b), hi = from_right((uint32_t)(b >> 32));
    return __longlong_as_double((long long)(((uint64_t)hi << 32) | lo));
}
__device__ __forceinline__ uint32_t ng_wet_rows(const unsigned long long *__restrict__ wet, int64_t rb, int64_t cc, int64_t H, int64_t W, int ntr, bool inner_col)
{
    const int t0 = ho::wet_tile_row(rb, ntr), t1 = t0 + 1 < ntr ? t0 + 1 : ntr - 1;
    const uint64_t w0 = wet[(int64_t)t0 * W + cc], w1 = wet[(int64_t)t1 * W + cc];
    return inner_col ? (uint32_t)ho::wet_rows64(w0, w1, 0ull, rb, H, ntr) : 0u;
}
template <bool D8, bool STORE = true, bool WET = false>
__global__ __launch_bounds__(256) void ng_finish_kernel(const float *__restrict__ F, const uint32_t *__restrict__ d, const float *__restrict__ dem,
                                                        double *__restrict__ G, int64_t H, int64_t W, double sh, double dg, double seed_add, int fixed_top,
                                                        int fixed_bot, unsigned long long *counters, uint8_t *__restrict__ flowdir, unsigned int *nodir,
                                                        const unsigned long long *__restrict__ wet, int ntr)
{
    const int lane = threadIdx.x & 63, wave = threadIdx.x >> 6;
    const int64_t c = ((int64_t)blockIdx.x * 4 + wave) * TI + lane - 1;
    const int64_t rb = (int64_t)blockIdx.y * FRB;
    const bool col_in = c >= 0 && c < W;
    const int64_t cc = c < 0 ? 0 : (c < W ? c : W - 1);
    const bool mine = lane >= 1 && lane <= TI && col_in;
    const bool inner_col = c > 0 && c + 1 < W;
    const double PINF = __builtin_inf();
    unsigned unreached = 0, bad = 0, anynodir = 0;
    float fb = 0.0f, fn = 0.0f;
    auto value = [&](int64_t r) -> double {
        if (!(r >= 0 && r < H && col_in)) return PINF;
        bool beyond;
        fn = F[r * W + cc];
        const double v = ng_value(fn, d[r * W + cc], seed_add, &beyond);
        unreached += beyond && mine && r >= rb && r < rb + FRB ? 1u : 0u;
        return v;
    };
    uint32_t wrows = 0u;
    if constexpr (WET) wrows = ng_wet_rows(wet, rb, cc, H, W, ntr, inner_col);
    double a = value(rb - 1), b = value(rb);
    fb = fn;
// ... 36 lines not shown

#ifndef NG_FINISH_AHEAD
#define NG_FINISH_AHEAD 1
#endif
#ifndef NG_FINISH_WAVES
#define NG_FINISH_WAVES 8
#endif
#if NG_FINISH_WAVES < 8
#define NG_FINISH_RESIDENCY __attribute__((amdgpu_waves_per_eu(1, NG_FINISH_WAVES)))
#else
#define NG_FINISH_RESIDENCY
#endif
#if NG_FINISH_AHEAD
template <bool STORE, bool WET>
__device__ __forceinline__ void ng_finish_ahead(const float *__restrict__ F, const uint32_t *__restrict__ d, const float *__restrict__ dem,
                                                double *__restrict__ G, int64_t H, int64_t W, double sh, double dg, double seed_add, int fixed_top,
                                                int fixed_bot, unsigned long long *counters, uint8_t *__restrict__ flowdir, unsigned int *nodir,
                                                const unsigned long long *__restrict__ wet, int ntr)
{
    const int lane = threadIdx.x & 63, wave = threadIdx.x >> 6;
    const int64_t c = ((int64_t)blockIdx.x * 4 + wave) * TI + lane - 1;
    const int64_t rb = (int64_t)blockIdx.y * FRB;
    const bool col_in = c >= 0 && c < W;
    const int64_t cc = c < 0 ? 0 : (c < W ? c : W - 1);
    const bool mine = lane >= 1 && lane <= TI && col_in;
    const bool inner_col = c > 0 && c + 1 < W;
    const double PINF = __builtin_inf();
    unsigned unreached = 0, bad = 0, anynodir = 0;
    struct RowZ {
        float f, z;
        uint32_t dd;
    };
    struct RowW {
        float f;
        uint32_t dd;
    };
    typedef typename std::conditional<WET, RowW, RowZ>::type Row;
    auto load = [&](int64_t r) -> Row {
        const int64_t at = (r < 0 ? 0 : (r < H ? r : H - 1)) * W + cc;
        if constexpr (WET) return Row{F[at], d[at]};
        else return Row{F[at], dem[at], d[at]};
    };
    uint32_t wrows = 0u;
    if constexpr (WET) wrows = ng_wet_rows(wet, rb, cc, H, W, ntr, inner_col);
    auto dem_of = [&](const Row &x) -> double {
        if constexpr (WET) {
            const double v = wrows & 1u ? -PINF : (double)x.f;
            wrows >>= 1;
            return v;
        } else
            return (double)x.z;
    };
    auto value = [&](int64_t r, const Row &x) -> double {
        if (!(r >= 0 && r < H && col_in)) return PINF;
        bool beyond;
        const double v = ng_value(x.f, x.dd, seed_add, &beyond);
        unreached += beyond && mine && r >= rb && r < rb + FRB ? 1u : 0u;
        return v;
    };
    const Row xa = load(rb - 1), xb = load(rb);
    Row x0 = load(rb + 1), x1{};
    double a = value(rb - 1, xa), b = value(rb, xb);
    double dvb = dem_of(xb);
    auto row = [&](int i, const Row &xn, Row &xnn, auto more) {
        const int64_t r = rb + i;
        const double dv = dvb;
        if (decltype(more)::value) xnn = load(r + 2);
        const double n = value(r + 1, xn);
        dvb = dem_of(xn);
        asm volatile("" : "+v"(dvb));
        const double al = dleft(a), ar = dright(a), bl = dleft(b), br = dright(b), nl = dleft(n), nr = dright(n);
        if (mine && r < H) {
            double want = dv;
            if (r > 0 && r < H - 1 && inner_col) {
                const double md = fmin(fmin(al, ar), fmin(nl, nr)) + dg;
                const double me = fmin(fmin(a, bl), fmin(br, n)) + sh;
                want = fmax(fmin(md, me), dv);
            }
            const bool halo = (r == 0 && fixed_top) || (r == H - 1 && fixed_bot);
            bad += (b == want || halo) ? 0u : 1u;
            if (STORE) G[r * W + c] = b;
            unsigned code;
            if (r == 0 || r == H - 1 || c == 0 || c == W - 1) code = edge_code(r, c, H - 1, W - 1);
            else {
                code = d8_code(b, a, ar, br, nr, n, nl, bl, al);
                anynodir |= code == 8u ? 1u : 0u;
            }
            flowdir[r * W + c] = (uint8_t)code;
        }
        a = b;
        b = n;
    };
    static_assert(FRB % 2 == 0, "rows in pairs");
    int i = 0;
    for (; i < FRB - 2 && rb + i < H; i += 2) {
        row(i, x0, x1, std::true_type());
        row(i + 1, x1, x0, std::true_type());
    }
    if (i == FRB - 2 && rb + i < H) {
        row(i, x0, x1, std::true_type());
        row(i + 1, x1, x0, std::false_type());
    }
    if (unreached) atomicAdd(&counters[C_UNREACHED], (unsigned long long)unreached);
    if (bad) atomicAdd(&counters[C_MISMATCH], (unsigned long long)bad);
    if (__any(anynodir != 0u) && lane == 0) *nodir = 1u;
}
#define NG_FINISH_AHEAD_KERNEL(STORE, WET)                                                                                                             \
    template <>                                                                                                                                        \
    __global__ __launch_bounds__(256) NG_FINISH_RESIDENCY void ng_finish_kernel<true, STORE, WET>(                                                     \
        const float *__restrict__ F, const uint32_t *__restrict__ d, const float *__restrict__ dem, double *__restrict__ G, int64_t H, int64_t W,      \
        double sh, double dg, double seed_add, int fixed_top, int fixed_bot, unsigned long long *counters, uint8_t *__restrict__ flowdir,              \
        unsigned int *nodir, const unsigned long long *__restrict__ wet, int ntr)                                                                      \
    {                                                                                                                                                  \
        ng_finish_ahead<STORE, WET>(F, d, dem, G, H, W, sh, dg, seed_add, fixed_top, fixed_bot, counters, flowdir, nodir, wet, ntr);                   \
    }
NG_FINISH_AHEAD_KERNEL(true, false)
NG_FINISH_AHEAD_KERNEL(false, false)
NG_FINISH_AHEAD_KERNEL(true, true)
NG_FINISH_AHEAD_KERNEL(false, true)
#undef NG_FINISH_AHEAD_KERNEL
#endif

uint32_t class_weight(double eps, int e)
{
    if (!(eps > 0.0) || std::isinf(eps)) return 0;
    int q;
    const double fr = std::frexp(eps, &q);
    const uint64_t M = (uint64_t)std::ldexp(fr, 53);
    const int k = (e - 127 - 52) - (q - 53);
    if (k <= 24 || k > 52) return 0;
    const uint64_t half = 1ull << (k - 1), rem = M & ((1ull << k) - 1);
    if (rem == half) return 0;
    const uint64_t w = (M >> k) + (rem > half ? 1 : 0);
    return (w >= 1 && w < WMAX) ? (uint32_t)w : 0;
}

}

struct GeoRun::Impl {
    DevBuf ws;
    uint32_t *d_tab = nullptr, *d_any = nullptr, *d_hdr = nullptr, *d_blk = nullptr;
    unsigned long long *d_cnt = nullptr;
    uint8_t *d_mark = nullptr;
    int *d_list = nullptr, *d_list2 = nullptr, *d_amark = nullptr;
    int ntr = 0, ntc = 0, round = 0, used = 0;
    std::vector<std::pair<hipEvent_t, hipEvent_t>> span;
    int span_rounds = 0;
    uint32_t last_count = 0xffffffffu;
    bool light = false;
    int light_from = 0;
    int64_t nt = 0;
    size_t lds = 0;
    int maxcyc = NG_MAXCYC;
    bool debug = false;
    unsigned long long irregular = 0;
};
namespace {
constexpr int MAXR = 8192, BATCH = 32, BATCH_HEAD = 16;
constexpr uint32_t LIGHT_TILES = 6144;
__global__ void ng_mark_row_kernel(uint8_t *mark, int ti, int ntc)
{
    const int tj = blockIdx.x * blockDim.x + threadIdx.x;
    if (tj < ntc) mark[(int64_t)ti * ntc + tj] = 1;
}
}

GeoRun::GeoRun() : impl(new Impl) {}
GeoRun::~GeoRun()
{
    for (auto &e : impl->span) {
        (void)hipEventDestroy(e.first);
        (void)hipEventDestroy(e.second);
    }
    delete impl;
}

int GeoRun::launch_rounds(hipStream_t s, int nb)
{
    {
        Impl &mm = *impl;
        hipEvent_t e0, e1;
        MH_HIP(hipEventCreate(&e0));
        MH_HIP(hipEventCreate(&e1));
        mm.span.emplace_back(e0, e1);
        MH_HIP(hipEventRecord(e0, s));
    }
    struct CloseSpan {
        Impl &m;
        hipStream_t s;
        ~CloseSpan() { (void)hipEventRecord(m.span.back().second, s); }
    } close_span{*impl, s};
    Impl &m = *impl;
    GeoArgs a;
    a.H = H; a.W = W; a.ntr = m.ntr; a.ntc = m.ntc; a.nt = (int)m.nt; a.F = filled; a.d = dist; a.tab = m.d_tab; a.counters = m.d_cnt;
    a.blk = m.d_blk; a.hdr = m.d_hdr; a.mark = m.d_mark; a.list = m.d_list; a.fixed_top = fixed_top; a.fixed_bot = fixed_bot;
    a.append = 0; a.round_next = 0; a.amark = m.d_amark; a.list_next = nullptr; a.count_next = nullptr;
    a.ho_dem = nullptr; a.ho_bslot = nullptr; a.ho_tabV = nullptr; a.ho_F = nullptr; a.ho_depths = nullptr; a.ho_wet = nullptr;
    const unsigned grid = (unsigned)std::min<int64_t>((m.nt + 3) / 4, 512);
    for (int k = 0; k < nb; ++k, ++m.round) {
        a.maxcyc = m.maxcyc;
        a.count = m.d_any + m.round;
        if (!m.round && handover && handover->pending) {
            a.ho_dem = handover->dem; a.ho_bslot = handover->bslot; a.ho_tabV = handover->tabV;
            a.ho_F = handover->filled; a.ho_depths = handover->depths; a.ho_wet = handover->wet;
            hipLaunchKernelGGL(ng_handover_kernel, dim3(grid), dim3(256), m.lds, s, a);
            handover->queued = true;
            (void)hipEventRecord(m.span.back().first, s);
            continue;
        }
        if (!m.round) {
            hipLaunchKernelGGL(ng_first_kernel, dim3(grid), dim3(256), m.lds, s, a);
            (void)hipEventRecord(m.span.back().first, s);
            continue;
        }
        if (!m.light || m.round == m.light_from)
            hipLaunchKernelGGL(ng_compact_kernel, dim3((unsigned)(((m.nt + 7) / 8 + 255) / 256)), dim3(256), 0, s, reinterpret_cast<unsigned long long *>(m.d_mark),
                               (int)((m.nt + 7) / 8), m.d_list, m.d_any + m.round);
        if (m.light) {
            const bool odd = ((m.round - m.light_from) & 1) != 0;
            a.append = 1;
            a.round_next = m.round + 1;
            a.list = odd ? m.d_list2 : m.d_list;
            a.list_next = odd ? m.d_list : m.d_list2;
            a.count_next = m.d_any + m.round + 1;
        }
        if (m.light && tail_hook && tail_hook->at == StageHook::TAIL_ROUNDS)
            hipLaunchKernelGGL(ng_round_w1_kernel, dim3((unsigned)std::min<int64_t>(m.nt, 2048)), dim3(64), (WN * (WN + 1) + 512) * sizeof(uint32_t), s, a);
        else
            hipLaunchKernelGGL(ng_round_kernel, dim3(grid), dim3(256), m.lds, s, a);
    }
    MH_HIP(hipGetLastError());
    return MHIP_OK;
}

int GeoRun::begin(hipStream_t s, bool *applicable, bool *active)
{
    Impl &m = *impl;
    static const bool off = [] { const char *e = dev_env("MHIP_NOFLAT"); return e && std::string(e) == "iterative"; }();
    m.debug = dev_env("MHIP_NG_DEBUG") != nullptr;
    *applicable = false;
    *active = false;
    if (off || !filled || H < 3 || W < 3) return MHIP_OK;
    if (!(sh > 0.0) || !(dg > 0.0) || std::isinf(sh) || std::isinf(dg)) return MHIP_OK;
    std::vector<uint32_t> tab(512, 0u);
    bool any_class = false;
    for (int e = 0; e < 255; ++e) {
        const uint32_t S = class_weight(sh, e), G = class_weight(dg, e);
        if (S && G) {
            tab[e] = S;
            tab[256 + e] = G;
            any_class = true;
        }
    }
    if (!any_class) return MHIP_OK;

    const int64_t n = H * W;
    m.ntr = (int)((H - 2 + TI - 1) / TI);
    m.ntc = (int)((W - 2 + TI - 1) / TI);
    m.nt = (int64_t)m.ntr * m.ntc;
    auto align = [](size_t x) { return (x + 255) & ~size_t(255); };
    const size_t o_d = 0, o_tab = align(o_d + (dist ? 0 : 4 * (size_t)n)), o_cnt = align(o_tab + 2048);
    const size_t o_any = align(o_cnt + 8 * (C_STATS + 128 + 16)), o_mark = align(o_any + 4 * (size_t)(MAXR + BATCH));
    const size_t o_amark = align(o_mark + (size_t)m.nt + 8), o_list = align(o_amark + 4 * (size_t)m.nt), o_list2 = align(o_list + 4 * (size_t)m.nt);
    const size_t o_hdr = align(o_list2 + 4 * (size_t)m.nt), o_blk = align(o_hdr + 4 * (size_t)m.nt);
    MH_TRY(m.ws.alloc(o_blk + 4 * (size_t)m.nt * WN * WN + 256));
    char *b = m.ws.as<char>();
    if (!dist) dist = reinterpret_cast<uint32_t *>(b + o_d);
    m.d_tab = reinterpret_cast<uint32_t *>(b + o_tab);
    m.d_cnt = reinterpret_cast<unsigned long long *>(b + o_cnt);
    m.d_any = reinterpret_cast<uint32_t *>(b + o_any);
    m.d_mark = reinterpret_cast<uint8_t *>(b + o_mark);
    m.d_list = reinterpret_cast<int *>(b + o_list);
    m.d_list2 = reinterpret_cast<int *>(b + o_list2);
    m.d_amark = reinterpret_cast<int *>(b + o_amark);
    m.d_hdr = reinterpret_cast<uint32_t *>(b + o_hdr);
    m.d_blk = reinterpret_cast<uint32_t *>(b + o_blk);
    MH_HIP(hipMemsetAsync(b + o_cnt, 0, o_list - o_cnt, s));
    MH_HIP(hipMemcpyAsync(m.d_tab, tab.data(), 2048, hipMemcpyHostToDevice, s));
    if (fixed_top) MH_HIP(hipMemsetAsync(dist, 0xE0, 4 * (size_t)W, s));
    if (fixed_bot) MH_HIP(hipMemsetAsync(dist + (H - 1) * W, 0xE0, 4 * (size_t)W, s));

    m.lds = (4 * WN * (WN + 1) + 512) * sizeof(uint32_t);
    {
        static std::mutex mu;
        static bool attr_done[64] = {};
        int dev = 0;
        MH_HIP(hipGetDevice(&dev));
        std::lock_guard<std::mutex> lk(mu);
        if (dev < 0 || dev >= 64 || !attr_done[dev]) {
            MH_HIP(hipFuncSetAttribute((const void *)ng_round_kernel, hipFuncAttributeMaxDynamicSharedMemorySize, (int)m.lds));
            MH_HIP(hipFuncSetAttribute((const void *)ng_first_kernel, hipFuncAttributeMaxDynamicSharedMemorySize, (int)m.lds));
            MH_HIP(hipFuncSetAttribute((const void *)ng_handover_kernel, hipFuncAttributeMaxDynamicSharedMemorySize, (int)m.lds));
            if (dev >= 0 && dev < 64) attr_done[dev] = true;
        }
    }
    m.round = 0;
    m.last_count = 0xffffffffu;
    m.used = 0;
    if (handover && handover->pending &&
        !(handover->ntr == m.ntr && handover->ntc == m.ntc && handover->H == H && handover->W == W && handover->filled == filled && handover->dem == dem &&
          !fixed_top && !fixed_bot))
        MH_TRY(fill_handover_complete(handover, s));
    const bool took = handover && handover->pending;
    MH_TRY(launch_rounds(s, 1));
    unsigned long long h_c[5] = {0, 0, 0, 0, 0};
    MH_HIP(hipMemcpyAsync(h_c, m.d_cnt, sizeof(h_c), hipMemcpyDeviceToHost, s));
    MH_HIP(stream_sync(s));
    if (took) {
        if (h_c[C_PROOF] != 0 || dev_env("MHIP_HO_RECHECK") != nullptr) {
            handover->suspect = true;
            m.ws.release();
            return MHIP_OK;
        }
        handover->release();
        handover->wet_ok = handover->wet != nullptr;
    }
    m.used = 1;
    m.irregular = h_c[C_IRREGULAR];
    if (h_c[C_FATAL] || (m.irregular && !allow_partial)) {
        if (m.debug) fprintf(stderr, "[noflat geodesic] %llu irregular flat cells, %llu NaN cells: float64 relaxation\n", m.irregular, h_c[C_FATAL]);
        return MHIP_OK;
    }
    *applicable = true;
    *active = true;
    return MHIP_OK;
}

int GeoRun::batch(hipStream_t s, bool *active)
{
    Impl &m = *impl;
    const char *eb = dev_env("MHIP_NG_BATCH");
    const int nb_env = eb && atoi(eb) >= 1 && atoi(eb) <= BATCH ? atoi(eb) : 0;
    for (;;) {
        const int nb = nb_env ? nb_env : (!m.light ? BATCH_HEAD : (m.last_count <= 64 ? 8 : (m.last_count <= 512 ? 16 : BATCH)));
        if (m.round + BATCH > MAXR) {
            set_error("no-flats fill (geodesic) did not converge within %d rounds", MAXR);
            return MHIP_ENOTCONV;
        }
        MH_TRY(launch_rounds(s, nb));
        if (tail_hook) tail_hook->fire_at(StageHook::TAIL_ROUNDS, s);
        uint32_t h_any[BATCH];
        MH_HIP(hipMemcpyAsync(h_any, m.d_any + (m.round - nb), sizeof(uint32_t) * nb, hipMemcpyDeviceToHost, s));
        MH_HIP(stream_sync(s));
        for (int k = 0; k < nb; ++k) {
            if (!h_any[k]) {
                *active = false;
                m.light = false;
                return MHIP_OK;
            }
            ++m.used;
        }
        m.last_count = h_any[nb - 1];
        if (!m.light && h_any[nb - 1] <= LIGHT_TILES) {
            m.light = true;
            m.light_from = m.round;
        }
    }
}

int GeoRun::halo_changed(int side, hipStream_t s)
{
    Impl &m = *impl;
    hipLaunchKernelGGL(ng_mark_row_kernel, dim3((unsigned)((m.ntc + 255) / 256)), dim3(256), 0, s, m.d_mark, side == 0 ? 0 : m.ntr - 1, m.ntc);
    MH_HIP(hipGetLastError());
    return MHIP_OK;
}

int GeoRun::end(hipStream_t s, bool *ok, FillStats *st)
{
    Impl &m = *impl;
    const int64_t n = H * W;
    partial = m.irregular != 0 && allow_partial;
    if (dev_env("MHIP_NG_CORRUPT") && W > 8)
        MH_HIP(hipMemsetAsync(dist + (H / 2) * W + 1, 0x01, 4 * (size_t)(W - 2), s));
    d8_done = false;
    const bool with_d8 = !partial && d8_out && d8_nodir && !fixed_top && !fixed_bot;
    if (tail_hook) tail_hook->fire_at(StageHook::FINISH, s);
    const bool no_store = with_d8 && defer_out;
    out_deferred = false;
    const unsigned long long *wet = handover && handover->wet_ok && !fixed_top && !fixed_bot ? handover->wet : nullptr;
    wet_used = false;
    const dim3 fgrid((unsigned)((W + 4 * TI - 1) / (4 * TI)), (unsigned)((H + FRB - 1) / FRB));
    auto finish = [&](auto d8_tag, auto store_tag, auto wet_tag, uint8_t *fd, unsigned int *nd) {
        hipLaunchKernelGGL((ng_finish_kernel<decltype(d8_tag)::value, decltype(store_tag)::value, decltype(wet_tag)::value>), fgrid, dim3(256), 0, s, filled, dist, dem,
                           out, H, W, sh, dg, seed_add, fixed_top, fixed_bot, m.d_cnt, fd, nd, wet, m.ntr);
        wet_used = decltype(wet_tag)::value;
    };
    const std::true_type yes;
    const std::false_type no;
    if (no_store && wet) finish(yes, no, yes, d8_out, d8_nodir);
    else if (no_store) finish(yes, no, no, d8_out, d8_nodir);
    else if (with_d8 && wet) finish(yes, yes, yes, d8_out, d8_nodir);
    else if (with_d8) finish(yes, yes, no, d8_out, d8_nodir);
    else if (!partial && wet) finish(no, yes, yes, nullptr, nullptr);
    else if (!partial) finish(no, yes, no, nullptr, nullptr);
    else
        hipLaunchKernelGGL(ng_assemble_kernel, dim3((unsigned)((n + 1023) / 1024)), dim3(256), 0, s, filled, dist, out, n, seed_add, m.d_cnt);
    MH_HIP(hipGetLastError());
    unsigned long long h_all[C_STATS + 128 + 16];
    MH_HIP(hipMemcpyAsync(h_all, m.d_cnt, sizeof(h_all), hipMemcpyDeviceToHost, s));
    MH_HIP(stream_sync(s));
    if (allow_partial && h_all[C_UNREACHED]) partial = true;
    if (st) {
        *st = FillStats();
        st->geo_irregular = (int64_t)m.irregular;
        st->geo_unreached = (int64_t)h_all[C_UNREACHED];
        st->geo_mismatch = (int64_t)h_all[C_MISMATCH];
        st->rounds = m.used;
        st->tiles = m.nt;
        st->algorithm = partial ? 3 : 2;
        for (auto &e : m.span) {
            float ms = 0;
            if (hipEventElapsedTime(&ms, e.first, e.second) == hipSuccess) st->hot_ms += ms;
            else (void)hipGetLastError();
        }
        st->hot_launches = m.used > 0 ? m.used - 1 : 0;
        for (int k = 0; k < 64; ++k) {
            st->visits += (int64_t)h_all[C_STATS + 2 * k];
            st->cycles += (int64_t)h_all[C_STATS + 2 * k + 1];
        }
    }
    if (m.debug) {
        std::vector<uint32_t> cnt((size_t)m.round);
        MH_HIP(hipMemcpy(cnt.data(), m.d_any, 4 * (size_t)m.round, hipMemcpyDeviceToHost));
        unsigned long long v = 0, cy = 0;
        for (int k = 0; k < 64; ++k) {
            v += h_all[C_STATS + 2 * k];
            cy += h_all[C_STATS + 2 * k + 1];
        }
        fprintf(stderr, "[noflat geodesic] tiles %lld, visits %llu, cycles %llu; tiles per round:", (long long)m.nt, v, cy);
        for (int k = 1; k < m.round && k < 200; ++k) fprintf(stderr, " %u", cnt[k]);
#ifdef NG_PROFILE
        for (int o = 0; o < 2; ++o) {
            const unsigned long long *q = h_all + C_STATS + 128 + 8 * o;
            if (q[0]) fprintf(stderr, "\n[noflat visits, %s] %llu: ticks per visit: setup+issue %.0f, wait for loads %.0f, relax %.0f, store %.0f", o ? "open" : "masked", q[0],
                              (double)q[1] / q[0], (double)q[2] / q[0], (double)q[3] / q[0], (double)q[4] / q[0]);
        }
#endif
        fprintf(stderr, "\n[noflat geodesic] %lld x %lld: rounds %d, unreached %llu, mismatches %llu\n", (long long)H, (long long)W, m.used, h_all[C_UNREACHED],
                h_all[C_MISMATCH]);
    }
    *ok = partial ? true : !(h_all[C_UNREACHED] || h_all[C_MISMATCH]);
    d8_done = with_d8 && !partial && *ok;
    if (no_store) {
        if (d8_done) out_deferred = true;
        else MH_TRY(noflat_assemble_dev(filled, dist, out, n, seed_add, s));
    }
    m.ws.release();
    return MHIP_OK;
}

int noflat_assemble_dev(const float *d_filled, const uint32_t *d_dist, double *d_out, int64_t n, double seed_add, hipStream_t s)
{
    hipLaunchKernelGGL(ng_assemble_kernel, dim3((unsigned)((n + 1023) / 1024)), dim3(256), 0, s, d_filled, d_dist, d_out, n, seed_add,
                       (unsigned long long *)nullptr);
    MH_HIP(hipGetLastError());
    return MHIP_OK;
}

int noflat_verify_dev(const float *d_dem, const double *d_out, int64_t H, int64_t W, double sh, double dg, hipStream_t s, bool *ok, int fixed_top,
                      int fixed_bot)
{
    DevBuf cnt;
    MH_TRY(cnt.alloc(8 * (C_STATS + 128 + 16)));
    MH_HIP(hipMemsetAsync(cnt.p, 0, 8 * (C_STATS + 128), s));
    hipLaunchKernelGGL(ng_verify_kernel, dim3((unsigned)((W + 255) / 256), (unsigned)((H + VRB - 1) / VRB)), dim3(256), 0, s, d_dem, d_out, H, W, sh, dg, fixed_top,
                       fixed_bot, cnt.as<unsigned long long>());
    MH_HIP(hipGetLastError());
    unsigned long long bad = 0;
    MH_HIP(hipMemcpyAsync(&bad, cnt.as<unsigned long long>() + C_MISMATCH, 8, hipMemcpyDeviceToHost, s));
    MH_HIP(stream_sync(s));
    *ok = bad == 0;
    return MHIP_OK;
}

int fill_noflat_geodesic_dev(const float *d_dem, const float *d_filled, double *d_out, int64_t H, int64_t W, double sh, double dg, double seed_add,
                             hipStream_t s, FillStats *st, bool *partial, StageHook *tail_hook, D8Sink *d8, FillHandover *ho)
{
    GeoRun g;
    g.handover = ho;
    g.tail_hook = tail_hook;
    if (d8) {
        g.d8_out = d8->flowdir; g.d8_nodir = d8->nodir; d8->done = false; d8->deferred = false;
        if (d8->dist) g.dist = d8->dist;
        g.defer_out = d8->defer && d8->dist;
    }
    g.dem = d_dem; g.filled = d_filled; g.out = d_out; g.H = H; g.W = W; g.sh = sh; g.dg = dg;
    g.allow_partial = partial != nullptr && seed_add == seed_add && seed_add < 1e300;
    g.seed_add = seed_add;
    bool applicable = false, active = false, ok = false;
    MH_TRY(g.begin(s, &applicable, &active));
    if (ho && ho->pending) {
        const bool again = ho->suspect;
        MH_TRY(fill_handover_complete(ho, s));
        if (again) {
            g.handover = nullptr;
            MH_TRY(g.begin(s, &applicable, &active));
        }
    }
    if (tail_hook) tail_hook->fire_at(StageHook::FIRST_VISIT, s);
    if (!applicable) {
        if (st) st->geo_reject = 1;
        return MHIP_ELIMIT;
    }
    while (active) MH_TRY(g.batch(s, &active));
    MH_TRY(g.end(s, &ok, st));
    if (partial) *partial = g.partial;
    if (d8) { d8->done = g.d8_done; d8->deferred = g.out_deferred; }
    if (ho) ho->wet_pass = g.wet_used;
    if (!ok && st) st->geo_reject = 2;
    return ok ? MHIP_OK : MHIP_ELIMIT;
}

}
```

Before: 13030 Mcells/s.

## Store only changed rows in noflat geodesic round kernels

The noflat geodesic round kernels now record which tile rows changed during relaxation and write back only those rows instead of the whole tile. Three modes are added: whole-tile, per-block-of-six-row tracking through separate accumulators, and per-row tracking in inline asm with a wave reduction. Block tracking is the default and can be chosen at runtime through an environment variable. The aim is to cut global store traffic on revisited tiles, at the cost of extra accumulators, ballots and register pressure inside the hot relax loop.

```diff
diff --git a/malstroem_amd/csrc/common.hpp b/malstroem_amd/csrc/common.hpp
--- a/malstroem_amd/csrc/common.hpp
+++ b/malstroem_amd/csrc/common.hpp
@@ -162,6 +162,8 @@
     float dem_min = 0.0f, dem_max = 0.0f;
     int32_t geo_reject = 0;
     int64_t geo_irregular = 0, geo_unreached = 0, geo_mismatch = 0;
+    int32_t rowstore = 0;
+    int64_t rows_stored = 0;
 };
 
 struct FillRun {
diff --git a/malstroem_amd/csrc/ctx.hip b/malstroem_amd/csrc/ctx.hip
--- a/malstroem_amd/csrc/ctx.hip
+++ b/malstroem_amd/csrc/ctx.hip
@@ -476,6 +476,8 @@
     else if (k == "noflat_reject_unreached") *value = c->noflat_st.geo_unreached;
     else if (k == "noflat_reject_mismatch") *value = c->noflat_st.geo_mismatch;
     else if (k == "noflat_cycles") *value = c->noflat_st.cycles;
+    else if (k == "noflat_rowstore") *value = c->noflat_st.rowstore;
+    else if (k == "noflat_rows_stored") *value = c->noflat_st.rows_stored;
     else if (k == "hyps_bins") *value = c->hyps_total;
     else if (k == "hyps_lds_spills") *value = c->hyps_spills;
     else if (k == "wet_at_events") *value = c->wetat_events;
diff --git a/malstroem_amd/csrc/noflat_geo.hip b/malstroem_amd/csrc/noflat_geo.hip
--- a/malstroem_amd/csrc/noflat_geo.hip
+++ b/malstroem_amd/csrc/noflat_geo.hip
@@ -27,6 +27,11 @@
 #define NG_MAXCYC 1
 #endif
 enum { C_IRREGULAR = 0, C_UNREACHED = 1, C_MISMATCH = 2, C_FATAL = 3, C_PROOF = 4, C_STATS = 8 };
+enum { C_ROWS = C_STATS + 128 + 16, C_END = C_ROWS + 64 };
+#ifndef NG_ROWSTORE
+#define NG_ROWSTORE 1
+#endif
+constexpr int NACC = 12;
 static_assert(WN == ho::WN && TI == ho::TI, "handover_addr.hpp cuts the raster like this file");
 
 __device__ __forceinline__ uint32_t from_left(uint32_t v) { return (uint32_t)__builtin_amdgcn_update_dpp(0, (int)v, DPP_WF_SR1, 0xf, 0xf, true); }
@@ -155,7 +160,7 @@
 
 template <typename WT>
 __device__ __forceinline__ void relax(uint32_t (&d)[WN], uint32_t (&ni)[WN], const WT wt, const uint32_t *tab_l, uint32_t scr_b, int lane, int maxcyc,
-                                      unsigned &wake, bool &changed, bool &capped, unsigned &cycles)
+                                      unsigned &wake, bool &changed, bool &capped, unsigned &cycles, uint64_t &rows)
 {
     const uint64_t INNER = ((1ull << TI) - 1) << 1, B1 = 2ull, B62 = 1ull << TI;
     capped = true;
@@ -170,6 +175,7 @@
             pass<false>(d, ni, wt, tab_l, acc_all, acc_first, acc_last);
             const uint64_t all = __ballot(acc_all != 0), fst = __ballot(acc_first != 0), lst = __ballot(acc_last != 0);
             chg |= all;
+            rows |= half == 0 ? (all ? ~0ull : 0ull) : all;
             const unsigned e_first = (fst & INNER) ? 1u : 0u, e_last = (lst & INNER) ? 1u : 0u;
             const unsigned l1 = (all & B1) ? 1u : 0u, l62 = (all & B62) ? 1u : 0u;
             const unsigned f1 = (fst & B1) ? 1u : 0u, f62 = (fst & B62) ? 1u : 0u, g1 = (lst & B1) ? 1u : 0u, g62 = (lst & B62) ? 1u : 0u;
@@ -190,6 +196,44 @@
 }
 
 constexpr int NMK = 9;
+__device__ __forceinline__ void lane_rows_of(const uint32_t (&rm_dn)[2], const uint32_t (&rm_up)[2], uint32_t (&lane_rows)[2])
+{
+    lane_rows[0] |= __builtin_bitreverse32(rm_dn[0]) | (rm_up[0] << 1);
+    lane_rows[1] |= (__builtin_bitreverse32(rm_dn[1]) >> 1) | rm_up[1];
+}
+__device__ __forceinline__ uint64_t wave_rows(const uint32_t (&lane_rows)[2], int lane)
+{
+    uint32_t lo = lane_rows[0], hi = lane_rows[1];
+    int at = lane << 2;
+    asm volatile("" : "+v"(at));
+#pragma unroll
+    for (int o = 32; o >= 1; o >>= 1) {
+        lo |= (uint32_t)__builtin_amdgcn_ds_bpermute(at ^ (o << 2), (int)lo);
+        hi |= (uint32_t)__builtin_amdgcn_ds_bpermute(at ^ (o << 2), (int)hi);
+    }
+    return (uint64_t)(uint32_t)__builtin_amdgcn_readfirstlane((int)lo) | ((uint64_t)(uint32_t)__builtin_amdgcn_readfirstlane((int)hi) << 32);
+}
+template <bool BLK> __device__ __forceinline__ constexpr int acc_of(int r) { return !BLK ? 0 : (r == 1 ? 0 : (r == TI ? NACC - 1 : 1 + (r - 2) / 6)); }
+template <bool BLK> __device__ __forceinline__ uint32_t acc_any(const uint32_t (&acc)[NACC])
+{
+    uint32_t v = acc[0];
+    if constexpr (BLK) {
+#pragma unroll
+        for (int k = 1; k < NACC; ++k) v |= acc[k];
+    }
+    return v;
+}
+template <bool BLK> __device__ __forceinline__ uint64_t block_rows(const uint32_t (&acc)[NACC], const uint64_t all)
+{
+    if constexpr (!BLK) return all ? ~0ull : 0ull;
+    uint64_t m = 0;
+#pragma unroll
+    for (int k = 0; k < NACC; ++k) {
+        const uint64_t rows_k = k == 0 ? 2ull : (k == NACC - 1 ? 1ull << TI : 0x3full << (2 + 6 * (k - 1)));
+        m |= __ballot(acc[k] != 0u) ? rows_k : 0ull;
+    }
+    return m;
+}
 #define NG_DPP " row_mask:0xf bank_mask:0xf bound_ctrl:1\n\t"
 #define NG_ROW(O, I, B, BIT)                                                                                                                 \
     "v_add_u32 %[u], %[" B "], %[S]\n\t"                                                                                                    \
@@ -200,76 +244,87 @@
     "v_min_u32 %[" O "], %[t], %[" I "]\n\t"                                                                                                \
     "v_bfi_b32 %[" O "], %[k], %[" I "], %[" O "]\n\t"                                                                                      \
     "v_bitop3_b32 %[acc], %[" O "], %[acc], %[" I "] bitop3:0xde\n\t"
-template <int R, int DIR>
-__device__ __forceinline__ void rows6_wl(uint32_t (&d)[WN], const uint32_t m, const uint32_t S, const uint32_t G, uint32_t &acc)
+#define NG_TRK(O, I)                                                                                                                         \
+    "v_cmp_ne_u32_e32 vcc, %[" O "], %[" I "]\n\t"                                                                                          \
+    "v_addc_co_u32_e32 %[rm], vcc, %[rm], %[rm], vcc\n\t"
+#define NG_ROW_T(O, I, B, BIT) NG_ROW(O, I, B, BIT) NG_TRK(O, I)
+#define NG_NONE
+#define NG_TRK_OUT , [rm] "+v"(rm)
+#define NG_TRK_CLOB : "vcc"
+#define NG_SIX(ROW, SGN) ROW("o0", "i0", "b", "%[bit]") ROW("o1", "i1", "o0", "%[bit]" SGN "1") ROW("o2", "i2", "o1", "%[bit]" SGN "2")       \
+    ROW("o3", "i3", "o2", "%[bit]" SGN "3") ROW("o4", "i4", "o3", "%[bit]" SGN "4") ROW("o5", "i5", "o4", "%[bit]" SGN "5")
+#define NG_SIX_OUT [o0] "=&v"(o0), [o1] "=&v"(o1), [o2] "=&v"(o2), [o3] "=&v"(o3), [o4] "=&v"(o4), [o5] "=&v"(o5), [u] "=&v"(u), [t] "=&v"(t), [k] "=&v"(k)
+#define NG_SIX_IN [b] "v"(d[R - DIR]), [i0] "v"(d[R]), [i1] "v"(d[R + DIR]), [i2] "v"(d[R + 2 * DIR]), [i3] "v"(d[R + 3 * DIR]), [i4] "v"(d[R + 4 * DIR]), [i5] "v"(d[R + 5 * DIR])
+#define NG_WL_SIX(ROW, SGN, XO, XC)                                                                                                          \
+    asm volatile(NG_SIX(ROW, SGN) : NG_SIX_OUT, [acc] "+v"(acc) XO : NG_SIX_IN, [S] "v"(S), [G] "v"(G), [m] "v"(m), [bit] "n"(R & 31) XC)
+#define NG_WL_ONE(ROW, XO, XC)                                                                                                               \
+    asm volatile("s_nop 1\n\t" ROW("o0", "i0", "b", "%[bit]") "s_nop 1"                                                                     \
+                 : [o0] "=&v"(o0), [u] "=&v"(u), [t] "=&v"(t), [k] "=&v"(k), [acc] "+v"(acc) XO                                               \
+                 : [b] "v"(d[R - DIR]), [i0] "v"(cu), [S] "v"(S), [G] "v"(G), [m] "v"(m), [bit] "n"(R & 31) XC)
+template <int R, int DIR, bool TRK>
+__device__ __forceinline__ void rows6_wl(uint32_t (&d)[WN], const uint32_t m, const uint32_t S, const uint32_t G, uint32_t &acc, uint32_t &rm)
 {
     static_assert((R >> 5) == ((R + 5 * DIR) >> 5), "one mask word a block");
     uint32_t o0, o1, o2, o3, o4, o5, u, t, k;
-    if constexpr (DIR > 0)
-        asm volatile(NG_ROW("o0", "i0", "b", "%[bit]") NG_ROW("o1", "i1", "o0", "%[bit]+1") NG_ROW("o2", "i2", "o1", "%[bit]+2")
-                     NG_ROW("o3", "i3", "o2", "%[bit]+3") NG_ROW("o4", "i4", "o3", "%[bit]+4") NG_ROW("o5", "i5", "o4", "%[bit]+5")
-                     : [o0] "=&v"(o0), [o1] "=&v"(o1), [o2] "=&v"(o2), [o3] "=&v"(o3), [o4] "=&v"(o4), [o5] "=&v"(o5), [u] "=&v"(u), [t] "=&v"(t),
-                       [k] "=&v"(k), [acc] "+v"(acc)
-                     : [b] "v"(d[R - DIR]), [i0] "v"(d[R]), [i1] "v"(d[R + DIR]), [i2] "v"(d[R + 2 * DIR]), [i3] "v"(d[R + 3 * DIR]),
-                       [i4] "v"(d[R + 4 * DIR]), [i5] "v"(d[R + 5 * DIR]), [S] "v"(S), [G] "v"(G), [m] "v"(m), [bit] "n"(R & 31));
-    else
-        asm volatile(NG_ROW("o0", "i0", "b", "%[bit]") NG_ROW("o1", "i1", "o0", "%[bit]-1") NG_ROW("o2", "i2", "o1", "%[bit]-2")
-                     NG_ROW("o3", "i3", "o2", "%[bit]-3") NG_ROW("o4", "i4", "o3", "%[bit]-4") NG_ROW("o5", "i5", "o4", "%[bit]-5")
-                     : [o0] "=&v"(o0), [o1] "=&v"(o1), [o2] "=&v"(o2), [o3] "=&v"(o3), [o4] "=&v"(o4), [o5] "=&v"(o5), [u] "=&v"(u), [t] "=&v"(t),
-                       [k] "=&v"(k), [acc] "+v"(acc)
-                     : [b] "v"(d[R - DIR]), [i0] "v"(d[R]), [i1] "v"(d[R + DIR]), [i2] "v"(d[R + 2 * DIR]), [i3] "v"(d[R + 3 * DIR]),
-                       [i4] "v"(d[R + 4 * DIR]), [i5] "v"(d[R + 5 * DIR]), [S] "v"(S), [G] "v"(G), [m] "v"(m), [bit] "n"(R & 31));
+    if constexpr (DIR > 0 && !TRK) NG_WL_SIX(NG_ROW, "+", NG_NONE, NG_NONE);
+    else if constexpr (DIR > 0) NG_WL_SIX(NG_ROW_T, "+", NG_TRK_OUT, NG_TRK_CLOB);
+    else if constexpr (!TRK) NG_WL_SIX(NG_ROW, "-", NG_NONE, NG_NONE);
+    else NG_WL_SIX(NG_ROW_T, "-", NG_TRK_OUT, NG_TRK_CLOB);
     d[R] = o0; d[R + DIR] = o1; d[R + 2 * DIR] = o2; d[R + 3 * DIR] = o3; d[R + 4 * DIR] = o4; d[R + 5 * DIR] = o5;
 }
-template <int R, int DIR>
-__device__ __forceinline__ uint32_t row1_wl(uint32_t (&d)[WN], const uint32_t m, const uint32_t S, const uint32_t G, uint32_t &acc)
+template <int R, int DIR, bool TRK>
+__device__ __forceinline__ uint32_t row1_wl(uint32_t (&d)[WN], const uint32_t m, const uint32_t S, const uint32_t G, uint32_t &acc, uint32_t &rm)
 {
     uint32_t o0, u, t, k;
     const uint32_t cu = d[R];
-    asm volatile("s_nop 1\n\t" NG_ROW("o0", "i0", "b", "%[bit]") "s_nop 1"
-                 : [o0] "=&v"(o0), [u] "=&v"(u), [t] "=&v"(t), [k] "=&v"(k), [acc] "+v"(acc)
-                 : [b] "v"(d[R - DIR]), [i0] "v"(cu), [S] "v"(S), [G] "v"(G), [m] "v"(m), [bit] "n"(R & 31));
+    if constexpr (!TRK) NG_WL_ONE(NG_ROW, NG_NONE, NG_NONE);
+    else NG_WL_ONE(NG_ROW_T, NG_TRK_OUT, NG_TRK_CLOB);
     d[R] = o0;
     return o0 ^ cu;
 }
-template <int R, int DIR, int N>
-__device__ __forceinline__ void blocks_wl(uint32_t (&d)[WN], const uint32_t lo, const uint32_t hi, const uint32_t S, const uint32_t G, uint32_t &acc)
+template <int R, int DIR, int N, bool BLK, bool TRK>
+__device__ __forceinline__ void blocks_wl(uint32_t (&d)[WN], const uint32_t lo, const uint32_t hi, const uint32_t S, const uint32_t G, uint32_t (&acc)[NACC],
+                                          uint32_t (&rm)[2])
 {
     if constexpr (N > 0) {
-        rows6_wl<R, DIR>(d, R < 32 ? lo : hi, S, G, acc);
+        rows6_wl<R, DIR, TRK>(d, R < 32 ? lo : hi, S, G, acc[acc_of<BLK>(R)], rm[R >> 5]);
         __builtin_amdgcn_sched_barrier(0);
-        blocks_wl<R + 6 * DIR, DIR, N - 1>(d, lo, hi, S, G, acc);
-    }
-}
-template <bool DOWN>
+        blocks_wl<R + 6 * DIR, DIR, N - 1, BLK, TRK>(d, lo, hi, S, G, acc, rm);
+    }
+}
+template <bool DOWN, bool BLK, bool TRK>
 __device__ __forceinline__ void pass_wl(uint32_t (&d)[WN], const uint32_t imm_lo, const uint32_t imm_hi, const uint32_t S, const uint32_t G,
-                                        const bool edge_first, const bool edge_last, uint32_t &acc_all, uint32_t &acc_first, uint32_t &acc_last)
+                                        const bool edge_first, const bool edge_last, uint32_t (&acc)[NACC], uint32_t (&rm)[2], uint32_t &acc_first,
+                                        uint32_t &acc_last)
 {
 #pragma unroll
     for (int r = 0; r < WN; ++r) asm volatile("" : "+v"(d[r]));
     uint32_t lo = imm_lo, hi = imm_hi;
     asm volatile("" : "+v"(lo), "+v"(hi));
     if constexpr (DOWN) {
-        const uint32_t x1 = row1_wl<1, 1>(d, lo, S, G, acc_all);
+        const uint32_t x1 = row1_wl<1, 1, TRK>(d, lo, S, G, acc[acc_of<BLK>(1)], rm[0]);
         acc_first |= edge_first ? x1 : 0u;
         __builtin_amdgcn_sched_barrier(0);
-        blocks_wl<2, 1, 10>(d, lo, hi, S, G, acc_all);
-        const uint32_t x2 = row1_wl<TI, 1>(d, hi, S, G, acc_all);
+        blocks_wl<2, 1, 10, BLK, TRK>(d, lo, hi, S, G, acc, rm);
+        const uint32_t x2 = row1_wl<TI, 1, TRK>(d, hi, S, G, acc[acc_of<BLK>(TI)], rm[1]);
         acc_last |= edge_last ? x2 : 0u;
     } else {
-        const uint32_t x2 = row1_wl<TI, -1>(d, hi, S, G, acc_all);
+        const uint32_t x2 = row1_wl<TI, -1, TRK>(d, hi, S, G, acc[acc_of<BLK>(TI)], rm[1]);
         acc_last |= edge_last ? x2 : 0u;
         __builtin_amdgcn_sched_barrier(0);
-        blocks_wl<TI - 1, -1, 10>(d, lo, hi, S, G, acc_all);
-        const uint32_t x1 = row1_wl<1, -1>(d, lo, S, G, acc_all);
+        blocks_wl<TI - 1, -1, 10, BLK, TRK>(d, lo, hi, S, G, acc, rm);
+        const uint32_t x1 = row1_wl<1, -1, TRK>(d, lo, S, G, acc[acc_of<BLK>(1)], rm[0]);
         acc_first |= edge_first ? x1 : 0u;
     }
     __builtin_amdgcn_sched_barrier(0);
 }
 
+template <int RS>
 __device__ __forceinline__ void relax_wl(uint32_t (&d)[WN], const uint32_t (&mk)[13], const uint32_t S, const uint32_t G, uint32_t scr_b, int lane, int maxcyc,
-                                         unsigned &wake, bool &changed, bool &capped, unsigned &cycles)
-{
+                                         unsigned &wake, bool &changed, bool &capped, unsigned &cycles, uint64_t &rows)
+{
+    constexpr bool BLK = RS == 1, TRK = RS == 2;
+    uint32_t lane_rows[2] = {0u, 0u};
     const uint64_t INNER = ((1ull << TI) - 1) << 1, B1 = 2ull, B62 = 1ull << TI;
     capped = true;
 #pragma nounroll
@@ -277,11 +332,13 @@
         uint64_t chg = 0;
         ++cycles;
         {
-            uint32_t acc_all = 0, acc_first = 0, acc_last = 0;
-            pass_wl<true>(d, mk[0], mk[1], S, G, (mk[8] & 1u) != 0u, (mk[8] & 2u) != 0u, acc_all, acc_first, acc_last);
-            pass_wl<false>(d, mk[0], mk[1], S, G, (mk[8] & 1u) != 0u, (mk[8] & 2u) != 0u, acc_all, acc_first, acc_last);
-            const uint64_t all = __ballot(acc_all != 0), fst = __ballot(acc_first != 0), lst = __ballot(acc_last != 0);
+            uint32_t acc[NACC] = {}, acc_first = 0, acc_last = 0, rm_dn[2] = {0u, 0u}, rm_up[2] = {0u, 0u};
+            pass_wl<true, BLK, TRK>(d, mk[0], mk[1], S, G, (mk[8] & 1u) != 0u, (mk[8] & 2u) != 0u, acc, rm_dn, acc_first, acc_last);
+            pass_wl<false, BLK, TRK>(d, mk[0], mk[1], S, G, (mk[8] & 1u) != 0u, (mk[8] & 2u) != 0u, acc, rm_up, acc_first, acc_last);
+            const uint64_t all = __ballot(acc_any<BLK>(acc) != 0), fst = __ballot(acc_first != 0), lst = __ballot(acc_last != 0);
             chg |= all;
+            if constexpr (TRK) lane_rows_of(rm_dn, rm_up, lane_rows);
+            else rows |= block_rows<BLK>(acc, all);
             const unsigned e_first = (fst & INNER) ? 1u : 0u, e_last = (lst & INNER) ? 1u : 0u;
             const unsigned l1 = (all & B1) ? 1u : 0u, l62 = (all & B62) ? 1u : 0u;
             const unsigned f1 = (fst & B1) ? 1u : 0u, f62 = (fst & B62) ? 1u : 0u, g1 = (lst & B1) ? 1u : 0u, g62 = (lst & B62) ? 1u : 0u;
@@ -289,11 +346,12 @@
             transpose32(d, scr_b, lane);
         }
         {
-            uint32_t acc_all = 0, acc_first = 0, acc_last = 0;
-            pass_wl<true>(d, mk[4], mk[5], S, G, (mk[8] & 4u) != 0u, (mk[8] & 8u) != 0u, acc_all, acc_first, acc_last);
-            pass_wl<false>(d, mk[4], mk[5], S, G, (mk[8] & 4u) != 0u, (mk[8] & 8u) != 0u, acc_all, acc_first, acc_last);
-            const uint64_t all = __ballot(acc_all != 0), fst = __ballot(acc_first != 0), lst = __ballot(acc_last != 0);
+            uint32_t acc[NACC] = {}, acc_first = 0, acc_last = 0, rm[2] = {0u, 0u};
+            pass_wl<true, false, false>(d, mk[4], mk[5], S, G, (mk[8] & 4u) != 0u, (mk[8] & 8u) != 0u, acc, rm, acc_first, acc_last);
+            pass_wl<false, false, false>(d, mk[4], mk[5], S, G, (mk[8] & 4u) != 0u, (mk[8] & 8u) != 0u, acc, rm, acc_first, acc_last);
+            const uint64_t all = __ballot(acc[0] != 0), fst = __ballot(acc_first != 0), lst = __ballot(acc_last != 0);
             chg |= all;
+            rows |= all;
             const unsigned e_first = (fst & INNER) ? 1u : 0u, e_last = (lst & INNER) ? 1u : 0u;
             const unsigned l1 = (all & B1) ? 1u : 0u, l62 = (all & B62) ? 1u : 0u;
             const unsigned f1 = (fst & B1) ? 1u : 0u, f62 = (fst & B62) ? 1u : 0u, g1 = (lst & B1) ? 1u : 0u, g62 = (lst & B62) ? 1u : 0u;
@@ -306,6 +364,7 @@
             break;
         }
     }
+    if constexpr (TRK) rows |= wave_rows(lane_rows, lane);
 }
 
 constexpr int NMK2 = 13;
@@ -324,80 +383,77 @@
 struct TwoWeights {
     uint32_t S1, G1, S2, G2;
 };
-template <int R, int DIR>
-__device__ __forceinline__ void rows6_wl2(uint32_t (&d)[WN], const uint32_t m, const uint32_t c, const TwoWeights w, uint32_t &acc)
+#define NG_ROW2_T(O, I, B, BIT) NG_ROW2(O, I, B, BIT) NG_TRK(O, I)
+#define NG_WL2_W [S1] "v"(w.S1), [G1] "v"(w.G1), [S2] "v"(w.S2), [G2] "v"(w.G2), [m] "v"(m), [c] "v"(c), [bit] "n"(R & 31)
+#define NG_WL2_SIX(ROW, SGN, XO, XC)                                                                                                         \
+    asm volatile(NG_SIX(ROW, SGN) : NG_SIX_OUT, [s] "=&v"(sw), [g] "=&v"(gw), [acc] "+v"(acc) XO : NG_SIX_IN, NG_WL2_W XC)
+#define NG_WL2_ONE(ROW, XO, XC)                                                                                                              \
+    asm volatile("s_nop 1\n\t" ROW("o0", "i0", "b", "%[bit]") "s_nop 1"                                                                     \
+                 : [o0] "=&v"(o0), [u] "=&v"(u), [t] "=&v"(t), [k] "=&v"(k), [s] "=&v"(sw), [g] "=&v"(gw), [acc] "+v"(acc) XO                 \
+                 : [b] "v"(d[R - DIR]), [i0] "v"(cu), NG_WL2_W XC)
+template <int R, int DIR, bool TRK>
+__device__ __forceinline__ void rows6_wl2(uint32_t (&d)[WN], const uint32_t m, const uint32_t c, const TwoWeights w, uint32_t &acc, uint32_t &rm)
 {
     static_assert((R >> 5) == ((R + 5 * DIR) >> 5), "one mask word a block");
     uint32_t o0, o1, o2, o3, o4, o5, u, t, k, sw, gw;
-    if constexpr (DIR > 0)
-        asm volatile(NG_ROW2("o0", "i0", "b", "%[bit]") NG_ROW2("o1", "i1", "o0", "%[bit]+1") NG_ROW2("o2", "i2", "o1", "%[bit]+2")
-                     NG_ROW2("o3", "i3", "o2", "%[bit]+3") NG_ROW2("o4", "i4", "o3", "%[bit]+4") NG_ROW2("o5", "i5", "o4", "%[bit]+5")
-                     : [o0] "=&v"(o0), [o1] "=&v"(o1), [o2] "=&v"(o2), [o3] "=&v"(o3), [o4] "=&v"(o4), [o5] "=&v"(o5), [u] "=&v"(u), [t] "=&v"(t),
-                       [k] "=&v"(k), [s] "=&v"(sw), [g] "=&v"(gw), [acc] "+v"(acc)
-                     : [b] "v"(d[R - DIR]), [i0] "v"(d[R]), [i1] "v"(d[R + DIR]), [i2] "v"(d[R + 2 * DIR]), [i3] "v"(d[R + 3 * DIR]),
-                       [i4] "v"(d[R + 4 * DIR]), [i5] "v"(d[R + 5 * DIR]), [S1] "v"(w.S1), [G1] "v"(w.G1), [S2] "v"(w.S2), [G2] "v"(w.G2), [m] "v"(m),
-                       [c] "v"(c), [bit] "n"(R & 31));
-    else
-        asm volatile(NG_ROW2("o0", "i0", "b", "%[bit]") NG_ROW2("o1", "i1", "o0", "%[bit]-1") NG_ROW2("o2", "i2", "o1", "%[bit]-2")
-                     NG_ROW2("o3", "i3", "o2", "%[bit]-3") NG_ROW2("o4", "i4", "o3", "%[bit]-4") NG_ROW2("o5", "i5", "o4", "%[bit]-5")
-                     : [o0] "=&v"(o0), [o1] "=&v"(o1), [o2] "=&v"(o2), [o3] "=&v"(o3), [o4] "=&v"(o4), [o5] "=&v"(o5), [u] "=&v"(u), [t] "=&v"(t),
-                       [k] "=&v"(k), [s] "=&v"(sw), [g] "=&v"(gw), [acc] "+v"(acc)
-                     : [b] "v"(d[R - DIR]), [i0] "v"(d[R]), [i1] "v"(d[R + DIR]), [i2] "v"(d[R + 2 * DIR]), [i3] "v"(d[R + 3 * DIR]),
-                       [i4] "v"(d[R + 4 * DIR]), [i5] "v"(d[R + 5 * DIR]), [S1] "v"(w.S1), [G1] "v"(w.G1), [S2] "v"(w.S2), [G2] "v"(w.G2), [m] "v"(m),
-                       [c] "v"(c), [bit] "n"(R & 31));
+    if constexpr (DIR > 0 && !TRK) NG_WL2_SIX(NG_ROW2, "+", NG_NONE, NG_NONE);
+    else if constexpr (DIR > 0) NG_WL2_SIX(NG_ROW2_T, "+", NG_TRK_OUT, NG_TRK_CLOB);
+    else if constexpr (!TRK) NG_WL2_SIX(NG_ROW2, "-", NG_NONE, NG_NONE);
+    else NG_WL2_SIX(NG_ROW2_T, "-", NG_TRK_OUT, NG_TRK_CLOB);
     d[R] = o0; d[R + DIR] = o1; d[R + 2 * DIR] = o2; d[R + 3 * DIR] = o3; d[R + 4 * DIR] = o4; d[R + 5 * DIR] = o5;
 }
-template <int R, int DIR>
-__device__ __forceinline__ uint32_t row1_wl2(uint32_t (&d)[WN], const uint32_t m, const uint32_t c, const TwoWeights w, uint32_t &acc)
+template <int R, int DIR, bool TRK>
+__device__ __forceinline__ uint32_t row1_wl2(uint32_t (&d)[WN], const uint32_t m, const uint32_t c, const TwoWeights w, uint32_t &acc, uint32_t &rm)
 {
     uint32_t o0, u, t, k, sw, gw;
     const uint32_t cu = d[R];
-    asm volatile("s_nop 1\n\t" NG_ROW2("o0", "i0", "b", "%[bit]") "s_nop 1"
-                 : [o0] "=&v"(o0), [u] "=&v"(u), [t] "=&v"(t), [k] "=&v"(k), [s] "=&v"(sw), [g] "=&v"(gw), [acc] "+v"(acc)
-                 : [b] "v"(d[R - DIR]), [i0] "v"(cu), [S1] "v"(w.S1), [G1] "v"(w.G1), [S2] "v"(w.S2), [G2] "v"(w.G2), [m] "v"(m), [c] "v"(c),
-                   [bit] "n"(R & 31));
+    if constexpr (!TRK) NG_WL2_ONE(NG_ROW2, NG_NONE, NG_NONE);
+    else NG_WL2_ONE(NG_ROW2_T, NG_TRK_OUT, NG_TRK_CLOB);
     d[R] = o0;
     return o0 ^ cu;
 }
-template <int R, int DIR, int N>
+template <int R, int DIR, int N, bool BLK, bool TRK>
 __device__ __forceinline__ void blocks_wl2(uint32_t (&d)[WN], const uint32_t lo, const uint32_t hi, const uint32_t clo, const uint32_t chi, const TwoWeights w,
-                                           uint32_t &acc)
+                                           uint32_t (&acc)[NACC], uint32_t (&rm)[2])
 {
     if constexpr (N > 0) {
-        rows6_wl2<R, DIR>(d, R < 32 ? lo : hi, R < 32 ? clo : chi, w, acc);
+        rows6_wl2<R, DIR, TRK>(d, R < 32 ? lo : hi, R < 32 ? clo : chi, w, acc[acc_of<BLK>(R)], rm[R >> 5]);
         __builtin_amdgcn_sched_barrier(0);
-        blocks_wl2<R + 6 * DIR, DIR, N - 1>(d, lo, hi, clo, chi, w, acc);
-    }
-}
-template <bool DOWN>
+        blocks_wl2<R + 6 * DIR, DIR, N - 1, BLK, TRK>(d, lo, hi, clo, chi, w, acc, rm);
+    }
+}
+template <bool DOWN, bool BLK, bool TRK>
 __device__ __forceinline__ void pass_wl2(uint32_t (&d)[WN], const uint32_t imm_lo, const uint32_t imm_hi, const uint32_t cls_lo, const uint32_t cls_hi,
-                                         const TwoWeights w, const bool edge_first, const bool edge_last, uint32_t &acc_all, uint32_t &acc_first,
-                                         uint32_t &acc_last)
+                                         const TwoWeights w, const bool edge_first, const bool edge_last, uint32_t (&acc)[NACC], uint32_t (&rm)[2],
+                                         uint32_t &acc_first, uint32_t &acc_last)
 {
 #pragma unroll
     for (int r = 0; r < WN; ++r) asm volatile("" : "+v"(d[r]));
     uint32_t lo = imm_lo, hi = imm_hi, clo = cls_lo, chi = cls_hi;
     asm volatile("" : "+v"(lo), "+v"(hi), "+v"(clo), "+v"(chi));
     if constexpr (DOWN) {
-        const uint32_t x1 = row1_wl2<1, 1>(d, lo, clo, w, acc_all);
+        const uint32_t x1 = row1_wl2<1, 1, TRK>(d, lo, clo, w, acc[acc_of<BLK>(1)], rm[0]);
         acc_first |= edge_first ? x1 : 0u;
         __builtin_amdgcn_sched_barrier(0);
-        blocks_wl2<2, 1, 10>(d, lo, hi, clo, chi, w, acc_all);
-        const uint32_t x2 = row1_wl2<TI, 1>(d, hi, chi, w, acc_all);
+        blocks_wl2<2, 1, 10, BLK, TRK>(d, lo, hi, clo, chi, w, acc, rm);
+        const uint32_t x2 = row1_wl2<TI, 1, TRK>(d, hi, chi, w, acc[acc_of<BLK>(TI)], rm[1]);
         acc_last |= edge_last ? x2 : 0u;
     } else {
-        const uint32_t x2 = row1_wl2<TI, -1>(d, hi, chi, w, acc_all);
+        const uint32_t x2 = row1_wl2<TI, -1, TRK>(d, hi, chi, w, acc[acc_of<BLK>(TI)], rm[1]);
         acc_last |= edge_last ? x2 : 0u;
         __builtin_amdgcn_sched_barrier(0);
-        blocks_wl2<TI - 1, -1, 10>(d, lo, hi, clo, chi, w, acc_all);
-        const uint32_t x1 = row1_wl2<1, -1>(d, lo, clo, w, acc_all);
+        blocks_wl2<TI - 1, -1, 10, BLK, TRK>(d, lo, hi, clo, chi, w, acc, rm);
+        const uint32_t x1 = row1_wl2<1, -1, TRK>(d, lo, clo, w, acc[acc_of<BLK>(1)], rm[0]);
         acc_first |= edge_first ? x1 : 0u;
     }
     __builtin_amdgcn_sched_barrier(0);
 }
+template <int RS>
 __device__ __forceinline__ void relax_wl2(uint32_t (&d)[WN], const uint32_t (&mk)[NMK2], const TwoWeights w, uint32_t scr_b, int lane, int maxcyc, unsigned &wake,
-                                          bool &changed, bool &capped, unsigned &cycles)
-{
+                                          bool &changed, bool &capped, unsigned &cycles, uint64_t &rows)
+{
+    constexpr bool BLK = RS == 1, TRK = RS == 2;
+    uint32_t lane_rows[2] = {0u, 0u};
     const uint64_t INNER = ((1ull << TI) - 1) << 1, B1 = 2ull, B62 = 1ull << TI;
     capped = true;
 #pragma nounroll
@@ -405,11 +461,13 @@
         uint64_t chg = 0;
         ++cycles;
         {
-            uint32_t acc_all = 0, acc_first = 0, acc_last = 0;
-            pass_wl2<true>(d, mk[0], mk[1], mk[9], mk[10], w, (mk[8] & 1u) != 0u, (mk[8] & 2u) != 0u, acc_all, acc_first, acc_last);
-            pass_wl2<false>(d, mk[0], mk[1], mk[9], mk[10], w, (mk[8] & 1u) != 0u, (mk[8] & 2u) != 0u, acc_all, acc_first, acc_last);
-            const uint64_t all = __ballot(acc_all != 0), fst = __ballot(acc_first != 0), lst = __ballot(acc_last != 0);
+            uint32_t acc[NACC] = {}, acc_first = 0, acc_last = 0, rm_dn[2] = {0u, 0u}, rm_up[2] = {0u, 0u};
+            pass_wl2<true, BLK, TRK>(d, mk[0], mk[1], mk[9], mk[10], w, (mk[8] & 1u) != 0u, (mk[8] & 2u) != 0u, acc, rm_dn, acc_first, acc_last);
+            pass_wl2<false, BLK, TRK>(d, mk[0], mk[1], mk[9], mk[10], w, (mk[8] & 1u) != 0u, (mk[8] & 2u) != 0u, acc, rm_up, acc_first, acc_last);
+            const uint64_t all = __ballot(acc_any<BLK>(acc) != 0), fst = __ballot(acc_first != 0), lst = __ballot(acc_last != 0);
             chg |= all;
+            if constexpr (TRK) lane_rows_of(rm_dn, rm_up, lane_rows);
+            else rows |= block_rows<BLK>(acc, all);
             const unsigned e_first = (fst & INNER) ? 1u : 0u, e_last = (lst & INNER) ? 1u : 0u;
             const unsigned l1 = (all & B1) ? 1u : 0u, l62 = (all & B62) ? 1u : 0u;
             const unsigned f1 = (fst & B1) ? 1u : 0u, f62 = (fst & B62) ? 1u : 0u, g1 = (lst & B1) ? 1u : 0u, g62 = (lst & B62) ? 1u : 0u;
@@ -417,11 +475,12 @@
             transpose32(d, scr_b, lane);
         }
         {
-            uint32_t acc_all = 0, acc_first = 0, acc_last = 0;
-            pass_wl2<true>(d, mk[4], mk[5], mk[11], mk[12], w, (mk[8] & 4u) != 0u, (mk[8] & 8u) != 0u, acc_all, acc_first, acc_last);
-            pass_wl2<false>(d, mk[4], mk[5], mk[11], mk[12], w, (mk[8] & 4u) != 0u, (mk[8] & 8u) != 0u, acc_all, acc_first, acc_last);
-            const uint64_t all = __ballot(acc_all != 0), fst = __ballot(acc_first != 0), lst = __ballot(acc_last != 0);
+            uint32_t acc[NACC] = {}, acc_first = 0, acc_last = 0, rm[2] = {0u, 0u};
+            pass_wl2<true, false, false>(d, mk[4], mk[5], mk[11], mk[12], w, (mk[8] & 4u) != 0u, (mk[8] & 8u) != 0u, acc, rm, acc_first, acc_last);
+            pass_wl2<false, false, false>(d, mk[4], mk[5], mk[11], mk[12], w, (mk[8] & 4u) != 0u, (mk[8] & 8u) != 0u, acc, rm, acc_first, acc_last);
+            const uint64_t all = __ballot(acc[0] != 0), fst = __ballot(acc_first != 0), lst = __ballot(acc_last != 0);
             chg |= all;
+            rows |= all;
             const unsigned e_first = (fst & INNER) ? 1u : 0u, e_last = (lst & INNER) ? 1u : 0u;
             const unsigned l1 = (all & B1) ? 1u : 0u, l62 = (all & B62) ? 1u : 0u;
             const unsigned f1 = (fst & B1) ? 1u : 0u, f62 = (fst & B62) ? 1u : 0u, g1 = (lst & B1) ? 1u : 0u, g62 = (lst & B62) ? 1u : 0u;
@@ -434,6 +493,7 @@
             break;
         }
     }
+    if constexpr (TRK) rows |= wave_rows(lane_rows, lane);
 }
 
 #define NG_ROW_OPEN(O, I, B)                                                                                                                 \
@@ -444,62 +504,69 @@
     "v_min_u32 %[" O "], %[t], %[" I "]\n\t"                                                                                                \
     "v_cndmask_b32_e64 %[" O "], %[" O "], %[" I "], %[ring]\n\t"                                                                            \
     "v_bitop3_b32 %[acc], %[" O "], %[acc], %[" I "] bitop3:0xde\n\t"
-template <int R, int DIR>
-__device__ __forceinline__ void rows6_open(uint32_t (&d)[WN], const uint64_t ring, const uint32_t S, const uint32_t G, uint32_t &acc)
-{
+#define NG_ROW_OPEN4(O, I, B, BIT) NG_ROW_OPEN(O, I, B)
+#define NG_ROW_OPEN_T(O, I, B, BIT) NG_ROW_OPEN(O, I, B) NG_TRK(O, I)
+#define NG_OPEN_SIX(ROW, XO, XC)                                                                                                             \
+    asm volatile(NG_SIX(ROW, "+") : NG_SIX_OUT, [acc] "+v"(acc) XO : NG_SIX_IN, [S] "v"(S), [G] "v"(G), [ring] "s"(ring) XC)
+#define NG_OPEN_ONE(ROW, XO, XC)                                                                                                             \
+    asm volatile("s_nop 1\n\t" ROW("o0", "i0", "b", "") "s_nop 1"                                                                           \
+                 : [o0] "=&v"(o0), [u] "=&v"(u), [t] "=&v"(t), [k] "=&v"(k), [acc] "+v"(acc) XO                                               \
+                 : [b] "v"(d[R - DIR]), [i0] "v"(cu), [S] "v"(S), [G] "v"(G), [ring] "s"(ring) XC)
+template <int R, int DIR, bool TRK>
+__device__ __forceinline__ void rows6_open(uint32_t (&d)[WN], const uint64_t ring, const uint32_t S, const uint32_t G, uint32_t &acc, uint32_t &rm)
+{
+    static_assert((R >> 5) == ((R + 5 * DIR) >> 5), "one mask word a block");
     uint32_t o0, o1, o2, o3, o4, o5, u, t, k;
-    asm volatile(NG_ROW_OPEN("o0", "i0", "b") NG_ROW_OPEN("o1", "i1", "o0") NG_ROW_OPEN("o2", "i2", "o1") NG_ROW_OPEN("o3", "i3", "o2")
-                 NG_ROW_OPEN("o4", "i4", "o3") NG_ROW_OPEN("o5", "i5", "o4")
-                 : [o0] "=&v"(o0), [o1] "=&v"(o1), [o2] "=&v"(o2), [o3] "=&v"(o3), [o4] "=&v"(o4), [o5] "=&v"(o5), [u] "=&v"(u), [t] "=&v"(t), [k] "=&v"(k),
-                   [acc] "+v"(acc)
-                 : [b] "v"(d[R - DIR]), [i0] "v"(d[R]), [i1] "v"(d[R + DIR]), [i2] "v"(d[R + 2 * DIR]), [i3] "v"(d[R + 3 * DIR]), [i4] "v"(d[R + 4 * DIR]),
-                   [i5] "v"(d[R + 5 * DIR]), [S] "v"(S), [G] "v"(G), [ring] "s"(ring));
+    if constexpr (!TRK) NG_OPEN_SIX(NG_ROW_OPEN4, NG_NONE, NG_NONE);
+    else NG_OPEN_SIX(NG_ROW_OPEN_T, NG_TRK_OUT, NG_TRK_CLOB);
     d[R] = o0; d[R + DIR] = o1; d[R + 2 * DIR] = o2; d[R + 3 * DIR] = o3; d[R + 4 * DIR] = o4; d[R + 5 * DIR] = o5;
 }
-template <int R, int DIR>
-__device__ __forceinline__ uint32_t row1_open(uint32_t (&d)[WN], const uint64_t ring, const uint32_t S, const uint32_t G, uint32_t &acc)
+template <int R, int DIR, bool TRK>
+__device__ __forceinline__ uint32_t row1_open(uint32_t (&d)[WN], const uint64_t ring, const uint32_t S, const uint32_t G, uint32_t &acc, uint32_t &rm)
 {
     uint32_t o0, u, t, k;
     const uint32_t cu = d[R];
-    asm volatile("s_nop 1\n\t" NG_ROW_OPEN("o0", "i0", "b") "s_nop 1"
-                 : [o0] "=&v"(o0), [u] "=&v"(u), [t] "=&v"(t), [k] "=&v"(k), [acc] "+v"(acc)
-                 : [b] "v"(d[R - DIR]), [i0] "v"(cu), [S] "v"(S), [G] "v"(G), [ring] "s"(ring));
+    if constexpr (!TRK) NG_OPEN_ONE(NG_ROW_OPEN4, NG_NONE, NG_NONE);
+    else NG_OPEN_ONE(NG_ROW_OPEN_T, NG_TRK_OUT, NG_TRK_CLOB);
     d[R] = o0;
     return o0 ^ cu;
 }
-template <int R, int DIR, int N>
-__device__ __forceinline__ void blocks_open(uint32_t (&d)[WN], const uint64_t ring, const uint32_t S, const uint32_t G, uint32_t &acc)
+template <int R, int DIR, int N, bool BLK, bool TRK>
+__device__ __forceinline__ void blocks_open(uint32_t (&d)[WN], const uint64_t ring, const uint32_t S, const uint32_t G, uint32_t (&acc)[NACC], uint32_t (&rm)[2])
 {
     if constexpr (N > 0) {
-        rows6_open<R, DIR>(d, ring, S, G, acc);
+        rows6_open<R, DIR, TRK>(d, ring, S, G, acc[acc_of<BLK>(R)], rm[R >> 5]);
         __builtin_amdgcn_sched_barrier(0);
-        blocks_open<R + 6 * DIR, DIR, N - 1>(d, ring, S, G, acc);
-    }
-}
-template <bool DOWN>
-__device__ __forceinline__ void pass_open(uint32_t (&d)[WN], const uint32_t S, const uint32_t G, const bool ring_lane, uint32_t &acc_all, uint32_t &acc_first,
-                                          uint32_t &acc_last)
+        blocks_open<R + 6 * DIR, DIR, N - 1, BLK, TRK>(d, ring, S, G, acc, rm);
+    }
+}
+template <bool DOWN, bool BLK, bool TRK>
+__device__ __forceinline__ void pass_open(uint32_t (&d)[WN], const uint32_t S, const uint32_t G, const bool ring_lane, uint32_t (&acc)[NACC], uint32_t (&rm)[2],
+                                          uint32_t &acc_first, uint32_t &acc_last)
 {
 #pragma unroll
     for (int r = 0; r < WN; ++r) asm volatile("" : "+v"(d[r]));
     const uint64_t ring = __ballot(ring_lane);
     if constexpr (DOWN) {
-        acc_first |= row1_open<1, 1>(d, ring, S, G, acc_all);
+        acc_first |= row1_open<1, 1, TRK>(d, ring, S, G, acc[acc_of<BLK>(1)], rm[0]);
         __builtin_amdgcn_sched_barrier(0);
-        blocks_open<2, 1, 10>(d, ring, S, G, acc_all);
-        acc_last |= row1_open<TI, 1>(d, ring, S, G, acc_all);
+        blocks_open<2, 1, 10, BLK, TRK>(d, ring, S, G, acc, rm);
+        acc_last |= row1_open<TI, 1, TRK>(d, ring, S, G, acc[acc_of<BLK>(TI)], rm[1]);
     } else {
-        acc_last |= row1_open<TI, -1>(d, ring, S, G, acc_all);
+        acc_last |= row1_open<TI, -1, TRK>(d, ring, S, G, acc[acc_of<BLK>(TI)], rm[1]);
         __builtin_amdgcn_sched_barrier(0);
-        blocks_open<TI - 1, -1, 10>(d, ring, S, G, acc_all);
-        acc_first |= row1_open<1, -1>(d, ring, S, G, acc_all);
+        blocks_open<TI - 1, -1, 10, BLK, TRK>(d, ring, S, G, acc, rm);
+        acc_first |= row1_open<1, -1, TRK>(d, ring, S, G, acc[acc_of<BLK>(1)], rm[0]);
     }
     __builtin_amdgcn_sched_barrier(0);
 }
 
+template <int RS>
 __device__ __forceinline__ void relax_open(uint32_t (&d)[WN], const uint32_t S, const uint32_t G, uint32_t scr_b, int lane, int maxcyc, unsigned &wake,
-                                           bool &changed, bool &capped, unsigned &cycles)
-{
+                                           bool &changed, bool &capped, unsigned &cycles, uint64_t &rows)
+{
+    constexpr bool BLK = RS == 1, TRK = RS == 2;
+    uint32_t lane_rows[2] = {0u, 0u};
     const uint64_t INNER = ((1ull << TI) - 1) << 1, B1 = 2ull, B62 = 1ull << TI;
     const bool ring_lane = (lane == 0) | (lane == WN - 1);
     capped = true;
@@ -509,11 +576,19 @@
         ++cycles;
 #pragma nounroll
         for (int half = 0; half < 2; ++half) {
-            uint32_t acc_all = 0, acc_first = 0, acc_last = 0;
-            pass_open<true>(d, S, G, ring_lane, acc_all, acc_first, acc_last);
-            pass_open<false>(d, S, G, ring_lane, acc_all, acc_first, acc_last);
-            const uint64_t all = __ballot(acc_all != 0), fst = __ballot(acc_first != 0), lst = __ballot(acc_last != 0);
+            uint32_t acc[NACC] = {}, acc_first = 0, acc_last = 0, rm_dn[2] = {0u, 0u}, rm_up[2] = {0u, 0u};
+            if (TRK && half == 0) {
+                pass_open<true, false, TRK>(d, S, G, ring_lane, acc, rm_dn, acc_first, acc_last);
+                pass_open<false, false, TRK>(d, S, G, ring_lane, acc, rm_up, acc_first, acc_last);
+                lane_rows_of(rm_dn, rm_up, lane_rows);
+            } else {
+                pass_open<true, BLK, false>(d, S, G, ring_lane, acc, rm_dn, acc_first, acc_last);
+                pass_open<false, BLK, false>(d, S, G, ring_lane, acc, rm_up, acc_first, acc_last);
+            }
+            const uint64_t all = __ballot(acc_any<BLK>(acc) != 0), fst = __ballot(acc_first != 0), lst = __ballot(acc_last != 0);
             chg |= all;
+            if (half == 1) rows |= all;
+            else if (!TRK) rows |= block_rows<BLK>(acc, all);
             const unsigned e_first = (fst & INNER) ? 1u : 0u, e_last = (lst & INNER) ? 1u : 0u;
             const unsigned l1 = (all & B1) ? 1u : 0u, l62 = (all & B62) ? 1u : 0u;
             const unsigned f1 = (fst & B1) ? 1u : 0u, f62 = (fst & B62) ? 1u : 0u, g1 = (lst & B1) ? 1u : 0u, g62 = (lst & B62) ? 1u : 0u;
@@ -527,12 +602,15 @@
             break;
         }
     }
+    if constexpr (TRK) rows |= wave_rows(lane_rows, lane);
 }
 
 constexpr uint32_t HDR_ACTIVE = 1u << 31, HDR_UNIFORM = 1u << 9, HDR_OPEN = 1u << 10, HDR_TWO = 1u << 11;
-template <bool FIRST, bool HANDOVER = false>
-__device__ __forceinline__ void visit(const GeoArgs &a, int t, const uint32_t *tab_l, uint32_t scr_b, int lane, unsigned &visits, unsigned &cycles)
-{
+template <bool FIRST, bool HANDOVER = false, int RS = 0>
+__device__ __forceinline__ void visit(const GeoArgs &a, int t, const uint32_t *tab_l, uint32_t scr_b, int lane, unsigned &visits, unsigned &cycles,
+                                      unsigned &rows_stored)
+{
+
 #ifdef NG_PROFILE
     const long long tp0 = __builtin_amdgcn_s_memtime();
 #endif
@@ -924,12 +1002,15 @@
     const uint32_t eref = (hdr >> 16) & 0xffu;
     unsigned wake = 0;
     bool changed = false, capped = false;
-    if (hdr & HDR_OPEN) relax_open(d, tab_l[eref], tab_l[256 + eref], scr_b, lane, a.maxcyc, wake, changed, capped, cycles);
+    uint64_t rows = 0;
+    bool walls = false;
+    if (hdr & HDR_OPEN) relax_open<RS>(d, tab_l[eref], tab_l[256 + eref], scr_b, lane, a.maxcyc, wake, changed, capped, cycles, rows);
     else if (hdr & HDR_UNIFORM) {
 #pragma unroll
         for (int r = 0; r < WN; ++r) d[r] |= (uint32_t)__builtin_amdgcn_sbfe((int)mk[2 + (r >> 5)], r & 31, 1) & DINF;
-        relax_wl(d, mk, tab_l[eref], tab_l[256 + eref], scr_b, lane, a.maxcyc, wake, changed, capped, cycles);
-        if (changed) {
+        relax_wl<RS>(d, mk, tab_l[eref], tab_l[256 + eref], scr_b, lane, a.maxcyc, wake, changed, capped, cycles, rows);
+        walls = true;
+        if (RS == 0 && changed) {
 #pragma unroll
             for (int r = 1; r <= TI; ++r) d[r] &= ~(uint32_t)__builtin_amdgcn_sbfe((int)mk[2 + (r >> 5)], r & 31, 1);
         }
@@ -938,12 +1019,13 @@
         const uint32_t c2 = (eref + ((hdr >> 24) & 0x7fu) - 64u) & 0xffu;
 #pragma unroll
         for (int r = 0; r < WN; ++r) d[r] |= (uint32_t)__builtin_amdgcn_sbfe((int)mk[2 + (r >> 5)], r & 31, 1) & DINF;
-        relax_wl2(d, mk, TwoWeights{tab_l[eref], tab_l[256 + eref], tab_l[c2], tab_l[256 + c2]}, scr_b, lane, a.maxcyc, wake, changed, capped, cycles);
-        if (changed) {
+        relax_wl2<RS>(d, mk, TwoWeights{tab_l[eref], tab_l[256 + eref], tab_l[c2], tab_l[256 + c2]}, scr_b, lane, a.maxcyc, wake, changed, capped, cycles, rows);
+        walls = true;
+        if (RS == 0 && changed) {
 #pragma unroll
             for (int r = 1; r <= TI; ++r) d[r] &= ~(uint32_t)__builtin_amdgcn_sbfe((int)mk[2 + (r >> 5)], r & 31, 1);
         }
-    } else relax(d, ni, LaneW{}, tab_l, scr_b, lane, a.maxcyc, wake, changed, capped, cycles);
+    } else relax(d, ni, LaneW{}, tab_l, scr_b, lane, a.maxcyc, wake, changed, capped, cycles, rows);
     wake &= hdr & 0x1ffu;
 #ifdef NG_PROFILE
     const long long tp3 = __builtin_amdgcn_s_memtime();
@@ -951,14 +1033,36 @@
 
     if (changed) {
         const bool lane_ok = (lane >= 1) & (lane <= TI) & (cc < W - 1);
-        if (lane_ok) {
-            if (last_row == WN - 1) {
-#pragma unroll
-                for (int r = 1; r <= TI; ++r) __builtin_amdgcn_raw_buffer_store_b32(d[r], rd, lane * 4, r * Wi * 4, 0);
-            } else {
-#pragma unroll
-                for (int r = 1; r <= TI; ++r)
-                    if (r < last_row) __builtin_amdgcn_raw_buffer_store_b32(d[r], rd, lane * 4, r * Wi * 4, 0);
+        const uint64_t mine = ((1ull << last_row) - 1ull) & ~1ull;
+        if constexpr (RS == 0) {
+            rows_stored += (unsigned)__builtin_popcountll(mine);
+            if (lane_ok) {
+                if (last_row == WN - 1) {
+#pragma unroll
+                    for (int r = 1; r <= TI; ++r) __builtin_amdgcn_raw_buffer_store_b32(d[r], rd, lane * 4, r * Wi * 4, 0);
+                } else {
+#pragma unroll
+                    for (int r = 1; r <= TI; ++r)
+                        if (r < last_row) __builtin_amdgcn_raw_buffer_store_b32(d[r], rd, lane * 4, r * Wi * 4, 0);
+                }
+            }
+        } else {
+            rows &= mine;
+            rows_stored += (unsigned)__builtin_popcountll(rows);
+            const uint32_t rows_lo = (uint32_t)rows, rows_hi = (uint32_t)(rows >> 32);
+            auto store_rows = [&](auto wall_tag) {
+#pragma unroll
+                for (int r = 1; r <= TI; ++r) {
+                    if (((r < 32 ? rows_lo : rows_hi) >> (r & 31)) & 1u) {
+                        uint32_t v = d[r];
+                        if constexpr (decltype(wall_tag)::value) v &= ~(uint32_t)__builtin_amdgcn_sbfe((int)mk[2 + (r >> 5)], r & 31, 1);
+                        __builtin_amdgcn_raw_buffer_store_b32(v, rd, lane * 4, r * Wi * 4, 0);
+                    }
+                }
+            };
+            if (lane_ok) {
+                if (walls) store_rows(std::true_type{});
+                else store_rows(std::false_type{});
             }
         }
     }
@@ -997,7 +1101,7 @@
 #endif
 }
 
-template <bool FIRST, int WPB = 4, bool HANDOVER = false>
+template <bool FIRST, int WPB = 4, bool HANDOVER = false, int RS = 0>
 __device__ __forceinline__ void round_body(const GeoArgs &a)
 {
     extern __shared__ __attribute__((aligned(16))) uint32_t lds[];
@@ -1014,20 +1118,30 @@
 #pragma unroll
     for (int k = 0; k < 512 / (64 * WPB); ++k) tab_l[threadIdx.x + k * 64 * WPB] = tw[k];
     __syncthreads();
-    unsigned visits = 0, cycles = 0;
+    unsigned visits = 0, cycles = 0, rows_stored = 0;
     for (int i = gw; i < n; i += nwaves) {
         const int t = FIRST ? i : __builtin_amdgcn_readfirstlane(i == gw ? t_first : a.list[i]);
-        visit<FIRST, HANDOVER>(a, t, tab_l, scr_b, lane, visits, cycles);
+        visit<FIRST, HANDOVER, RS>(a, t, tab_l, scr_b, lane, visits, cycles, rows_stored);
     }
     if (lane == 0 && visits) {
         unsigned long long *st = a.counters + C_STATS + 2 * (gw & 63);
         atomicAdd(&st[0], (unsigned long long)visits);
         atomicAdd(&st[1], (unsigned long long)cycles);
+        if (!FIRST && rows_stored) atomicAdd(&a.counters[C_ROWS + (gw & 63)], (unsigned long long)rows_stored);
     }
 }
 __global__ __launch_bounds__(256, 2) void ng_first_kernel(GeoArgs a) { round_body<true>(a); }
-__global__ __launch_bounds__(256, 2) void ng_round_kernel(GeoArgs a) { round_body<false>(a); }
-__global__ __launch_bounds__(64, 2) void ng_round_w1_kernel(GeoArgs a) { round_body<false, 1>(a); }
+__global__ __launch_bounds__(256, 2) void ng_round_kernel(GeoArgs a) { round_body<false, 4, false, NG_ROWSTORE>(a); }
+__global__ __launch_bounds__(64, 2) void ng_round_w1_kernel(GeoArgs a) { round_body<false, 1, false, NG_ROWSTORE>(a); }
+template <int RS> __global__ __launch_bounds__(256, 2) void ng_round_alt_kernel(GeoArgs a) { round_body<false, 4, false, RS>(a); }
+template <int RS> __global__ __launch_bounds__(64, 2) void ng_round_alt_w1_kernel(GeoArgs a) { round_body<false, 1, false, RS>(a); }
+typedef void (*RoundKernel)(GeoArgs);
+template <int RS> RoundKernel round_kernel(bool w1)
+{
+    if constexpr (RS == NG_ROWSTORE) return w1 ? ng_round_w1_kernel : ng_round_kernel;
+    else return w1 ? ng_round_alt_w1_kernel<RS> : ng_round_alt_kernel<RS>;
+}
+RoundKernel round_kernel(int rs, bool w1) { return rs == 0 ? round_kernel<0>(w1) : (rs == 1 ? round_kernel<1>(w1) : round_kernel<2>(w1)); }
 __global__ __launch_bounds__(256, 2) void ng_handover_kernel(GeoArgs a) { round_body<true, 4, true>(a); }
 
 __global__ __launch_bounds__(256) void ng_compact_kernel(unsigned long long *mark8, int nwords, int *list, uint32_t *count)
@@ -1370,6 +1484,7 @@
     int64_t nt = 0;
     size_t lds = 0;
     int maxcyc = NG_MAXCYC;
+    int rowstore = NG_ROWSTORE;
     bool debug = false;
     unsigned long long irregular = 0;
 };
@@ -1443,9 +1558,10 @@
             a.count_next = m.d_any + m.round + 1;
         }
         if (m.light && tail_hook && tail_hook->at == StageHook::TAIL_ROUNDS)
-            hipLaunchKernelGGL(ng_round_w1_kernel, dim3((unsigned)std::min<int64_t>(m.nt, 2048)), dim3(64), (WN * (WN + 1) + 512) * sizeof(uint32_t), s, a);
+            hipLaunchKernelGGL(round_kernel(m.rowstore, true), dim3((unsigned)std::min<int64_t>(m.nt, 2048)), dim3(64),
+                               (WN * (WN + 1) + 512) * sizeof(uint32_t), s, a);
         else
-            hipLaunchKernelGGL(ng_round_kernel, dim3(grid), dim3(256), m.lds, s, a);
+            hipLaunchKernelGGL(round_kernel(m.rowstore, false), dim3(grid), dim3(256), m.lds, s, a);
     }
     MH_HIP(hipGetLastError());
     return MHIP_OK;
@@ -1456,6 +1572,10 @@
     Impl &m = *impl;
     static const bool off = [] { const char *e = dev_env("MHIP_NOFLAT"); return e && std::string(e) == "iterative"; }();
     m.debug = dev_env("MHIP_NG_DEBUG") != nullptr;
+    {
+        const char *e = dev_env("MHIP_NG_ROWSTORE");
+        m.rowstore = e && e[0] >= '0' && e[0] <= '2' && !e[1] ? e[0] - '0' : NG_ROWSTORE;
+    }
     *applicable = false;
     *active = false;
     if (off || !filled || H < 3 || W < 3) return MHIP_OK;
@@ -1478,7 +1598,7 @@
     m.nt = (int64_t)m.ntr * m.ntc;
     auto align = [](size_t x) { return (x + 255) & ~size_t(255); };
     const size_t o_d = 0, o_tab = align(o_d + (dist ? 0 : 4 * (size_t)n)), o_cnt = align(o_tab + 2048);
-    const size_t o_any = align(o_cnt + 8 * (C_STATS + 128 + 16)), o_mark = align(o_any + 4 * (size_t)(MAXR + BATCH));
+    const size_t o_any = align(o_cnt + 8 * C_END), o_mark = align(o_any + 4 * (size_t)(MAXR + BATCH));
     const size_t o_amark = align(o_mark + (size_t)m.nt + 8), o_list = align(o_amark + 4 * (size_t)m.nt), o_list2 = align(o_list + 4 * (size_t)m.nt);
     const size_t o_hdr = align(o_list2 + 4 * (size_t)m.nt), o_blk = align(o_hdr + 4 * (size_t)m.nt);
     MH_TRY(m.ws.alloc(o_blk + 4 * (size_t)m.nt * WN * WN + 256));
@@ -1506,7 +1626,8 @@
         MH_HIP(hipGetDevice(&dev));
         std::lock_guard<std::mutex> lk(mu);
         if (dev < 0 || dev >= 64 || !attr_done[dev]) {
-            MH_HIP(hipFuncSetAttribute((const void *)ng_round_kernel, hipFuncAttributeMaxDynamicSharedMemorySize, (int)m.lds));
+            for (int rs = 0; rs <= 2; ++rs)
+                MH_HIP(hipFuncSetAttribute((const void *)round_kernel(rs, false), hipFuncAttributeMaxDynamicSharedMemorySize, (int)m.lds));
             MH_HIP(hipFuncSetAttribute((const void *)ng_first_kernel, hipFuncAttributeMaxDynamicSharedMemorySize, (int)m.lds));
             MH_HIP(hipFuncSetAttribute((const void *)ng_handover_kernel, hipFuncAttributeMaxDynamicSharedMemorySize, (int)m.lds));
             if (dev >= 0 && dev < 64) attr_done[dev] = true;
@@ -1615,7 +1736,7 @@
     else
         hipLaunchKernelGGL(ng_assemble_kernel, dim3((unsigned)((n + 1023) / 1024)), dim3(256), 0, s, filled, dist, out, n, seed_add, m.d_cnt);
     MH_HIP(hipGetLastError());
-    unsigned long long h_all[C_STATS + 128 + 16];
+    unsigned long long h_all[C_END];
     MH_HIP(hipMemcpyAsync(h_all, m.d_cnt, sizeof(h_all), hipMemcpyDeviceToHost, s));
     MH_HIP(stream_sync(s));
     if (allow_partial && h_all[C_UNREACHED]) partial = true;
@@ -1636,17 +1757,21 @@
         for (int k = 0; k < 64; ++k) {
             st->visits += (int64_t)h_all[C_STATS + 2 * k];
             st->cycles += (int64_t)h_all[C_STATS + 2 * k + 1];
-        }
+            st->rows_stored += (int64_t)h_all[C_ROWS + k];
+        }
+        st->rowstore = m.rowstore;
     }
     if (m.debug) {
         std::vector<uint32_t> cnt((size_t)m.round);
         MH_HIP(hipMemcpy(cnt.data(), m.d_any, 4 * (size_t)m.round, hipMemcpyDeviceToHost));
-        unsigned long long v = 0, cy = 0;
+        unsigned long long v = 0, cy = 0, rw = 0;
         for (int k = 0; k < 64; ++k) {
             v += h_all[C_STATS + 2 * k];
             cy += h_all[C_STATS + 2 * k + 1];
-        }
-        fprintf(stderr, "[noflat geodesic] tiles %lld, visits %llu, cycles %llu; tiles per round:", (long long)m.nt, v, cy);
+            rw += h_all[C_ROWS + k];
+        }
+        fprintf(stderr, "[noflat geodesic] tiles %lld, visits %llu, cycles %llu, rows stored %llu (row store %d); tiles per round:", (long long)m.nt, v, cy, rw,
+                m.rowstore);
         for (int k = 1; k < m.round && k < 200; ++k) fprintf(stderr, " %u", cnt[k]);
 #ifdef NG_PROFILE
         for (int o = 0; o < 2; ++o) {
```

After: 13160 Mcells/s, median of 6. +1.0%, better.
